# cjac/cmusphinx

Measured on AMD Instinct MI355X. Metric: decoded_frames_per_sec (full mode-4 decode, hub4-shaped CD-GMM 6144x8x39 + 20k-word lextrees + trigram; xRT = value/100/n_gpus), higher is better.
Workload: dtype f32-sub/f64-acc/int32-logadd (bit-exact), int32 Viterbi + word level; 1 GPU; lanes_per_gpu=512, engines_per_gpu=1

## Files before the change

### cmusphinx_amd/csrc/s3a_decoder_kernels.h

```cpp
#ifndef S3A_DECODER_KERNELS_H
#define S3A_DECODER_KERNELS_H
#include <hip/hip_runtime.h>
#include <stdlib.h>
#include <stdint.h>
#include <limits.h>
#include "s3a_device.h"
#include "s3a_structs.h"
#include "s3a_vit.h"
#include "s3a_scan.h"

#define WORST S3A_WORST
#define DBLOCK 256
#define S3A_ALD(p) __hip_atomic_load((p), __ATOMIC_RELAXED, __HIP_MEMORY_SCOPE_AGENT)
#define S3A_ALDU(p) __hip_atomic_load((p), __ATOMIC_RELAXED, __HIP_MEMORY_SCOPE_AGENT)
#define SCAN_LONG_LIST 16384
static inline int32_t scan_workgroups(int32_t rows, int chained)
{
    return (rows >= SCAN_LONG_LIST || chained) ? (rows + SCAN_THREADS - 1) / SCAN_THREADS : 1;
}
#define M3BLOCK 64
#define RSBLOCK 64
#define EVBLOCK_LONG_LIST 32768

struct FrameBeams {
// ... 1222 lines not shown
        c = lo;
        v = rootlist[calls[4 * c + 2] + (e - calls[4 * c + 3])];
    }
};

__device__ __forceinline__ void
d_dec_enter1(Entries ent, int32_t n_ent, const int32_t *__restrict__ calls,
             const int32_t *__restrict__ prob, const int32_t *__restrict__ sc, int32_t thresh,
             unsigned long long *key, int32_t *first,
        const int32_t BX, const int32_t BY)
{
    const int32_t e = BX * blockDim.x + threadIdx.x;
    int32_t idx, c;
    ent.locate_idx_wave(e < n_ent ? e : 0, idx, c);
    if (e >= n_ent) return;
    const int32_t scr = add32(calls[4 * c], ent.root_prob(idx, prob));
    if (scr < thresh) return;
    const int32_t v = ent.rootlist[idx];
    if (!(sc[NSV(v)] < scr)) return;
    atomicMax(&key[v], ((unsigned long long)((uint32_t)scr ^ 0x80000000u) << 32) | (uint32_t)(0x7fffffff - c));
    atomicMin(&first[v], c);
}

template <bool MAXOP>
__device__ __forceinline__ void
d_comsen_wave(int32_t n_cs, const int32_t *__restrict__ cs_need, int32_t stamp, const int32_t *__restrict__ cs_off,
              const int16_t *__restrict__ cs_list, uint8_t *sen_active, const int32_t *__restrict__ raw, int32_t *cs_val,
              int32_t cs0)
{
    const int32_t lane = threadIdx.x & 63, sub = lane >> 4, l16 = lane & 15;
    const int32_t mine = cs0 + lane;
    const unsigned long long mask = __ballot(mine < n_cs && cs_need[mine] == stamp);
    const int32_t n = __popcll(mask);
    for (int32_t k0 = 0; k0 < n; k0 += 4) {
        const int32_t k = k0 + sub;
        unsigned long long m = mask;
        for (int32_t i = 0; i < k && m; i++) m &= m - 1ull;
        const bool on = k < n;
        const int32_t cs = on ? cs0 + (__ffsll((long long)m) - 1) : 0;
        int32_t mx = INT_MIN;
        if (on)
            for (int32_t q = cs_off[cs] + l16, hi = cs_off[cs + 1]; q < hi; q += 16) {
                const int32_t id = cs_list[q];
                if (MAXOP) mx = max(mx, raw[id]); else sen_active[id] = 1;
            }
        if (MAXOP) {
#pragma unroll
            for (int o = 8; o > 0; o >>= 1) mx = max(mx, __shfl_xor(mx, o, 64));
            if (on && l16 == 0) cs_val[cs] = mx;
        }
    }
}

template <bool MAXOP, int U = 4>
__device__ __forceinline__ void
d_comsen_list(const int32_t *__restrict__ wl, int32_t n_w, const int32_t *__restrict__ cs_off, const int16_t *__restrict__ cs_list,
              uint8_t *sen_active, const int32_t *__restrict__ raw, int32_t *cs_val, int32_t grp, int32_t n_grp,
              const int32_t *__restrict__ cs_wt = NULL, uint32_t *actbits = NULL)
{
    const int32_t l16 = threadIdx.x & 15;
    for (int32_t j0 = 0; j0 < n_w; j0 += U * n_grp) {
        int32_t cs[U], lo[U], hi[U], mx[U];
        bool on[U];
#pragma unroll
        for (int u = 0; u < U; u++) { const int32_t j = j0 + u * n_grp + grp; on[u] = j < n_w; cs[u] = ((const __attribute__((address_space(1))) int32_t *)wl)[on[u] ? j : 0]; }
#pragma unroll
        for (int u = 0; u < U; u++) { const __attribute__((address_space(1))) int32_t *co = (const __attribute__((address_space(1))) int32_t *)cs_off; const int32_t a0 = co[cs[u]], a1 = co[cs[u] + 1]; lo[u] = on[u] ? a0 : 0; hi[u] = on[u] ? a1 : 0; mx[u] = INT_MIN; }
        for (int32_t q0 = 0; ; q0 += 32) {
            int32_t id[U][2];
            bool any = false;
#pragma unroll
            for (int u = 0; u < U; u++) {
#pragma unroll
                for (int h = 0; h < 2; h++) { const int32_t q = lo[u] + q0 + 16 * h + l16; const int32_t x = (int32_t)((const __attribute__((address_space(1))) int16_t *)cs_list)[q < hi[u] ? q : 0]; id[u][h] = q < hi[u] ? x : -1; }
                any = any || lo[u] + q0 < hi[u];
            }
            if (!any) break;
#pragma unroll
            for (int u = 0; u < U; u++)
#pragma unroll
                for (int h = 0; h < 2; h++)
                {
                    if (MAXOP) { const int32_t x = ((const __attribute__((address_space(1))) int32_t *)raw)[max(id[u][h], 0)]; if (id[u][h] >= 0) mx[u] = max(mx[u], x); }
                    else if (id[u][h] >= 0) { if (actbits) (void)__hip_atomic_fetch_or((__attribute__((address_space(3))) uint32_t *)&actbits[id[u][h] >> 5], 1u << (id[u][h] & 31), __ATOMIC_RELAXED, __HIP_MEMORY_SCOPE_WORKGROUP); else sen_active[id[u][h]] = 1; }
                }
        }
        if (MAXOP) {
#pragma unroll
            for (int u = 0; u < U; u++) {
#pragma unroll
                for (int o = 8; o > 0; o >>= 1) mx[u] = max(mx[u], __shfl_xor(mx[u], o, 64));
                if (on[u] && l16 == 0) ((__attribute__((address_space(1))) int32_t *)cs_val)[cs[u]] = cs_wt ? add32(mx[u], ((const __attribute__((address_space(1))) int32_t *)cs_wt)[cs[u]]) : mx[u];
            }
        }
    }
}

__device__ __forceinline__ void
mark_node_senones(int32_t v, const int32_t *__restrict__ ssid, const uint8_t *__restrict__ comp,
                  const int16_t *__restrict__ sseq, const int16_t *__restrict__ comsseq,
                  const int32_t *__restrict__ cs_off, const int16_t *__restrict__ cs_list, uint8_t *sen_active,
                  int32_t *cs_need = NULL, int32_t stamp = 0, int32_t ne = 3, int32_t *cs_wl = NULL, int32_t *cs_wn = NULL)
{
    const int32_t ss = ssid[v];
    if (comp[v] && cs_need && cs_wl) {
        for (int st = 0; st < ne; st++) {
            const int32_t cs = comsseq[ss * ne + st];
            if (atomicExch(&cs_need[cs], stamp) != stamp) cs_wl[atomicAdd(cs_wn, 1)] = cs;
        }
    }
    else if (comp[v] && cs_need) {
        if (ne == 3) {
#pragma unroll
            for (int st = 0; st < 3; st++) cs_need[comsseq[ss * 3 + st]] = stamp;
        }
        else for (int st = 0; st < ne; st++) cs_need[comsseq[ss * ne + st]] = stamp;
    }
    else if (comp[v] && ne != 3) {
        for (int st = 0; st < ne; st++) {
            const int32_t cs = comsseq[ss * ne + st];
            for (int32_t q = cs_off[cs]; q < cs_off[cs + 1]; q++) sen_active[cs_list[q]] = 1;
        }
    }
    else if (comp[v]) {
        int32_t lo[3], hi[3];
#pragma unroll
        for (int st = 0; st < 3; st++) {
            const int32_t cs = comsseq[ss * 3 + st];
            lo[st] = cs_off[cs]; hi[st] = cs_off[cs + 1];
        }
        while (lo[0] < hi[0] || lo[1] < hi[1] || lo[2] < hi[2]) {
            int32_t id[3][8];
#pragma unroll
            for (int st = 0; st < 3; st++)
#pragma unroll
                for (int u = 0; u < 8; u++) id[st][u] = (lo[st] + u < hi[st]) ? (int32_t)cs_list[lo[st] + u] : -1;
// ... 132 lines not shown
```

### cmusphinx_amd/csrc/s3a_utt.hip

```cpp
#include <hip/hip_runtime.h>
#include <stdint.h>
#include <stdlib.h>
#include <stdio.h>
#include <string.h>
#include <limits.h>
#include <vector>
#include <deque>
#include <atomic>
#include <mutex>
#include <algorithm>
#include <fcntl.h>
#include <unistd.h>
#include <sys/file.h>
#include <sys/stat.h>

#include "s3a_device.h"
#include "s3a_structs.h"
#include "s3a_decoder_kernels.h"
#include "s3a_gated.h"
#include "s3a_wordlevel.h"
#include "s3a_lm3g.h"
#include "s3a_dag.h"
#include "s3a_hostmem.h"
#include "s3a_kfplan.h"
#include "s3a_uttgeom.h"
#include "s3a_qsched.h"

#define S3A_AS1 __attribute__((address_space(1)))
#define S3A_AS3 __attribute__((address_space(3)))
typedef int s3a_v4i __attribute__((ext_vector_type(4)));
typedef int s3a_v2i __attribute__((ext_vector_type(2)));
template <class T> __device__ __forceinline__ S3A_AS1 T *GM(T *p) { return (S3A_AS1 T *)p; }
template <class T> __device__ __forceinline__ const S3A_AS1 T *GMC(const T *p) { return (const S3A_AS1 T *)p; }
template <class T> __device__ __forceinline__ const S3A_AS3 T *LM(const T *p) { return (const S3A_AS3 T *)p; }
__device__ __forceinline__ void lds_or(uint32_t *p, uint32_t v) { (void)__hip_atomic_fetch_or((S3A_AS3 uint32_t *)p, v, __ATOMIC_RELAXED, __HIP_MEMORY_SCOPE_WORKGROUP); }

struct ULane {
    int32_t *sc, *hist, *outs, *outh, *bests, *frame, *pos, *posf, *act[2], *nact[2], *turn, *selfemit, *cnt, *base,
        *best, *exits, *nexit, *first, *eflag, *hbin, *done, *ctot, *n0, *pstamp, *propf, *poswid, *posout, *scan_flag;
    unsigned long long *scan_agg, *scan_pre, *key;
    uint8_t *sen_act;
    int32_t *scr, *misc, *bstidx, *bstscr, *updatetime, *gpart;
    int32_t *cs_need, *cs_val;
    int32_t *cs_wl, *cs_wn;
    int32_t *posbest;
    uint32_t *senbits;
    int32_t *posps;
    int32_t *ent;
    uint8_t *pstamp8;
    int32_t *dynbeam;
    int32_t *claim;
    int32_t *plist, *pcnt;
    int32_t *win;
    uint8_t *winb;
    int32_t *ci_all;
    int32_t *heur_all;
    int32_t *hth_pos;
    int32_t *ph_scratch;
    UCtx *ctx;
    int32_t *pack;
    WLane w;
};

struct UShared {
    int32_t N, T, n_tmat, maxn, n_rootnodes, scan_chunks, pack_max_exits, gp_n, n_cs, n_pset_bytes;
    int32_t ne;
    const int32_t *node_base, *ssid, *tmatid, *wid, *prob, *child_off, *child, *par_off, *par, *tree_of, *rootlist, *tp,
        *rootnodes, *ps, *psof_off, *psof, *psmem_off, *psmem, *cs_off, *cs_wt, *rootprob;
    const uint8_t *comp;
    const int16_t *sseq, *comsseq, *cs_list;
    const int4 *node4;
    const int32_t *nodesen;
    const int4 *pshdr;
    const int4 *nodepk;
    const float4 *mean4, *prec4;
    const float *lrd;
    const int32_t *mixw;
    const uint16_t *tab16;
    uint32_t tab_size;
    int32_t lm_zero;
    double f, distfloor;
    int32_t D4, CP, Gpad, n_sen, n_ci_sen;
    const uint8_t *ncomp;
    const int16_t *cd2cisen;
    int32_t ds_ratio, ci_pbeam, ci_pbeam_tight, ptranskip;
    int32_t max_cd;
    float tighten;
    FrameBeams bm;
    int32_t pheurtype, pl_beam, pl_window, n_ci;
    const uint8_t *node_ci;
    const int16_t *sen2cimap;
    int32_t win_K;
    UCtx *ctx_all;
    int32_t *nact_all;
    const int32_t *fgbase;
};

#define LANE UCtx *ctx = S.ctx_all + blockIdx.z; const int32_t f = fg + *S.fgbase - ctx->f0;                         \
    if (f < 0 || f >= ctx->nfr || !ctx->active) return;                                                           \
    const int32_t cur = f & 1; const int32_t *nact_cur = S.nact_all + ((size_t)blockIdx.z * 2 + cur) * WL_MAXT;       \
    const ULane &L = lanes[blockIdx.z]; (void)cur; (void)nact_cur
#define SCR_ROW (S.win_K > 0 ? L.win + (size_t)(f % S.win_K) * S.n_sen : L.scr)

__device__ __forceinline__ FrameBeams
frame_beams(const UShared &S, int32_t cf)
{
    FrameBeams bm = S.bm;
    bm.phone_uses_wbeam = (S.ptranskip != 0 && (cf % S.ptranskip) == 0) ? 1 : 0;
    return bm;
}

struct UBegin { int32_t e0[10], lmc[5], n_pset; };

__device__ __forceinline__ void
// ... 564 lines not shown
            const int32_t sq = in ? senq[u] : S.n_ci_sen;
            actq[u] = actbits ? (uint8_t)((LM(actbits)[sq >> 5] >> (sq & 31)) & 1u) : L.sen_act[sq];
            if (!in) actq[u] = 0;
            ciq[u] = GMC(S.cd2cisen)[sq];
            senq[u] = sq;
        }
#pragma unroll
        for (int u = 0; u < 4; u++) {
            cisq[u] = GMC(row)[ciq[u]]; rowq[u] = GMC(row)[senq[u]]; nbq[u] = GMC(brow)[senq[u]];
            obq[u] = GMC(L.bstidx)[senq[u]]; utq[u] = GMC(L.updatetime)[senq[u]];
        }
#pragma unroll
        for (int u = 0; u < 4; u++) {
            if (!actq[u]) continue;
            const int32_t sen = senq[u];
            if (!actbits) L.sen_act[sen] = 0;
            const int32_t ci_scr = cisq[u];
            if (ci_scr >= thresh) {
                const int32_t bi = (int32_t)nbq[u];
                GM(L.bstidx)[sen] = bi == 255 ? S3A_NO_BSTIDX : bi;
                GM(L.updatetime)[sen] = f;
                rbest = max(rbest, rowq[u]); rns++; rng += (int32_t)GMC(S.ncomp)[sen];
                continue;
            }
            const int32_t bi = obq[u], ut = utq[u];
            if (bi == S3A_NO_BSTIDX || ut != f - 1) {
                GM(row)[sen] = ci_scr;
                rbest = max(rbest, ci_scr);
                continue;
            }
            const int32_t v = uw_one_gaussian<EXACT>(S, sen * S.CP + bi, ctx->feat + (size_t)f * S.D4 * 4);
            int32_t score = la(S3A_LOGPROB_ZERO, v);
            if (score <= S3A_LOGPROB_ZERO) score = S3A_LOGPROB_ZERO;
            row[sen] = score;
            rbest = max(rbest, score); rng++;
            if (is_skip) { L.bstidx[sen] = v > S3A_LOGPROB_ZERO ? bi : S3A_NO_BSTIDX; L.updatetime[sen] = f; }
        }
    }
#pragma unroll
    for (int o = 32; o > 0; o >>= 1) {
        rbest = max(rbest, __shfl_xor(rbest, o, 64)); rns += __shfl_xor(rns, o, 64); rng += __shfl_xor(rng, o, 64);
    }
    __syncthreads();
    if (ln == 0) { red[0][tid >> 6] = rbest; red[1][tid >> 6] = rns; red[2][tid >> 6] = rng; }
    __syncthreads();
    if (tid == 0 && bx < S.gp_n) {
        for (int w = 1; w < NT / 64; w++) { rbest = max(rbest, red[0][w]); rns += red[1][w]; rng += red[2][w]; }
        L.gpart[bx] = rbest;
        L.gpart[S.gp_n + bx] = rns;
        L.gpart[2 * S.gp_n + bx] = rng;
    }
}

template <bool EXACT>
__global__ void __launch_bounds__(256)
ku_select(const ULane *__restrict__ lanes, UShared S, int32_t fg, int32_t K)
{
    LANE;
    d_select<EXACT, 256>(L, S, ctx, f, L.win + (size_t)(f % K) * S.n_sen, L.winb + (size_t)(f % K) * S.n_sen, blockIdx.x, gridDim.x);
}

__global__ void __launch_bounds__(256)
ku_comsen_mark(const ULane *__restrict__ lanes, UShared S, int32_t fg)
{
    LANE;
    d_comsen_wave<false>(S.n_cs, L.cs_need, f, S.cs_off, S.cs_list, L.sen_act, (const int32_t *)NULL, (int32_t *)NULL,
                         (int32_t)blockIdx.x * 256 + (int32_t)(threadIdx.x & ~63));
}

#define UDB_MAXCI 1024
__global__ void __launch_bounds__(1024)
ku_dyn_ci_beam(const ULane *__restrict__ lanes, UShared S, int32_t fg)
{
    __shared__ int32_t s_occ[UDB_MAXCI], s_scr[UDB_MAXCI], s_ord[UDB_MAXCI], s_cut;
    LANE;
    const int32_t n_ci = S.n_ci_sen, tid = threadIdx.x;
    for (int32_t c = tid; c < n_ci; c += 1024) { s_occ[c] = 0; s_scr[c] = SCR_ROW[c]; }
    if (tid == 0) s_cut = INT_MAX;
    __syncthreads();
    for (int32_t s = n_ci + tid; s < S.n_sen; s += 1024)
        if (L.sen_act[s]) atomicAdd(&s_occ[S.cd2cisen[s]], 1);
    __syncthreads();
    for (int32_t c = tid; c < n_ci; c += 1024) {
        const int32_t v = s_scr[c];
        int32_t r = 0;
        for (int32_t c2 = 0; c2 < n_ci; c2++) { const int32_t v2 = s_scr[c2]; r += (v2 > v || (v2 == v && c2 < c)) ? 1 : 0; }
        s_ord[r] = c;
    }
    __syncthreads();
    const int32_t pbest = s_scr[s_ord[0]];
    for (int32_t r = tid; r < n_ci; r += 1024) {
        int32_t total = 0;
        for (int32_t r2 = 0; r2 <= r; r2++) total += s_occ[s_ord[r2]];
        if (total > S.max_cd) atomicMin(&s_cut, r);
    }
    __syncthreads();
    if (tid == 0) {
        int32_t beam = S.ci_pbeam;
        if (s_cut != INT_MAX) {
            const int32_t v = s_scr[s_ord[s_cut]];
            bool in_beam = true;
            for (int32_t r = 0; r <= s_cut && in_beam; r++) in_beam = s_scr[s_ord[r]] > add32(pbest, S.ci_pbeam);
            if (in_beam) beam = v - pbest;
        }
        if (f % S.ds_ratio != 0) beam = (int32_t)((float)beam * S.tighten);
        L.dynbeam[0] = beam;
// ... 568 lines not shown
#define KF_SENBITS 16384
#ifndef KF_ER
#define KF_ER 4
#endif
#ifndef KF_RL
#define KF_RL 8
#endif
#ifndef KF_SK
#define KF_SK 8
#endif
#ifndef KF_RK
#define KF_RK 4
#endif
#define KF_SETS 512
#define KF_TP_LDS 1024
#define KF_ENT 640
#define KF_BIG 256
static_assert(KF_NT == 512, "ku_frames: the word level's workgroup is the frame's workgroup");
enum { KF_WINDOW, KF_STATIC, KF_QUEUE };
#define KF_ST_WORDS 8
#define KF_OVERLAP_LEAD 128
#define KF_STAGES 2

union KfPool {
    struct { int32_t off[WL_MAXCALL], root[WL_MAXCALL], in[WL_MAXCALL], hist[WL_MAXCALL]; } e1;
    int32_t bin[NBIN];
    HistSortWs<KF_NT> hs;
    struct {
        union {
            int32_t rc[KF_WAVES][5 * 64];
            int32_t ent[KF_ENT][5];
        };
        int32_t mlo[KF_SETS], pre[KF_SETS + 1], big[KF_SETS], nbig, m_all;
        int32_t bmlo[KF_BIG], bnm[KF_BIG], bkp0[KF_BIG], bnp[KF_BIG];
        int32_t bnq[KF_BIG], bpre[KF_BIG + 1], bmpre[KF_BIG + 1], leg[KF_BIG], nleg;
        int32_t n_ent;
    } rs;
    struct { int32_t hdr[6 * WL_MAXT + 16], ex[3 * WL_LDS_EX]; } wl;
};

struct KfSh {
    KfPool pool;
    int32_t best[2 * WL_MAXT], acc[2 * WL_MAXT], pre[WL_MAXT + 1], red[KF_WAVES], dead, u, u2, dynbeam;
    int32_t fk, fk2;
    ULane Lc;
    int32_t nb[WL_MAXT + 1];
    int32_t seg[KF_MAXSEG + 1], ws[KF_WAVES + 1], gq[4];
    int32_t rk[KF_RK][KF_WAVES];
    uint32_t senbits[KF_SENBITS / 32];
    int32_t pstab[KF_PSTAB];
    int32_t ps_exact;
    uint32_t psbits[KF_PSBITS / 32];
    long long kacc[16];
    int32_t thr[4];
    int32_t tp[KF_TP_LDS];
    struct { const void *A; UCtx *ctx; int32_t *row; const uint8_t *brow; int32_t *bar_cnt; int32_t z, r, C, f, weak, bar_target, bar_local; } fa;
};

struct KfBar { int32_t *cnt; int32_t C, target; int32_t *dead; int32_t local; };

struct KfJob {
    int32_t mode, fg0, n_fr;
    int32_t n_utt;
    int32_t u0;
    const int32_t *order;
    int32_t stop_at;
    int32_t resume;
    int32_t *st_cur, *st_next;
    int32_t *lane_f, *lane_uq, *lane_stop;
    int32_t *next;
    int32_t *lane_u;
    const UCtx *stage;
    const long long *row0;
    int32_t *scores;
    const uint8_t *bests;
    int32_t *hdr, *words, *wcount;
    UHypPar P;
    UBegin B;
    int32_t n_word;
    int32_t ov;
    int32_t n1;
    const int32_t *q_ready;
    int32_t *lane_left;
    int32_t *n_resumed;
    const int32_t *f_ready;
    int32_t *n_inside;
};

__device__ __forceinline__ void
kf_barrier(KfBar &B)
{
    if (B.C == 1) { __syncthreads(); return; }
    if (B.local) asm volatile("s_waitcnt vmcnt(0) lgkmcnt(0)" ::: "memory");
    __syncthreads();
    B.target += B.C;
    if (threadIdx.x == 0 && !*B.dead) {
        if (!B.local) __builtin_amdgcn_fence(__ATOMIC_RELEASE, "agent");
        asm volatile("s_waitcnt vmcnt(0)" ::: "memory");
        (void)__hip_atomic_fetch_add(B.cnt, 1, __ATOMIC_RELAXED, __HIP_MEMORY_SCOPE_AGENT);
        int32_t spins = 0;
        while (__hip_atomic_load(B.cnt, __ATOMIC_RELAXED, __HIP_MEMORY_SCOPE_AGENT) < B.target) {
            __builtin_amdgcn_s_sleep(1);
            if (++spins > KF_SPIN_MAX) { *B.dead = 1; break; }
        }
        __builtin_amdgcn_fence(__ATOMIC_ACQUIRE, "agent");
    }
    __syncthreads();
}

__device__ __forceinline__ void
kf_locate(const int32_t *pre, int32_t T, int32_t g, int32_t &t, int32_t &i)
{
    t = 0;
    while (t + 1 < T && g >= pre[t + 1]) t++;
    i = g - pre[t];
}

template <int NE>
__device__ __forceinline__ int32_t
kf_hmm_eval(int32_t v, const int4 nd, const int32_t *__restrict__ nodesen, const int32_t *__restrict__ tp_g, const int32_t *tp_lds, const bool tp_in_lds,
            const int32_t *__restrict__ raw, const int32_t *raw_lds, const bool raw_in_lds, int32_t norm,
            const int32_t *__restrict__ cs_valw, int32_t *rec_all, int32_t cf, int32_t &w, int32_t &out)
{
    constexpr int NV = NE == 3 ? 2 : 3;
    S3A_AS1 s3a_v4i *rec = (S3A_AS1 s3a_v4i *)(rec_all + NSV(v));
    int32_t id[NE], tmat, wid_, comp;
    if (NE == 3) {
        id[0] = nd.x & 0xffff; id[1] = (int32_t)((uint32_t)nd.x >> 16); id[2] = nd.y & 0xffff;
        tmat = (int32_t)((uint32_t)nd.y >> 16); wid_ = nd.z; comp = nd.w & 1;
    }
    else {
        const s3a_v4i a5 = *(const S3A_AS1 s3a_v4i *)(nodesen + (size_t)v * 4);
        const int32_t h[5] = { a5.x & 0xffff, (int32_t)((uint32_t)a5.x >> 16), a5.y & 0xffff, (int32_t)((uint32_t)a5.y >> 16), a5.z & 0xffff };
#pragma unroll
        for (int st = 0; st < NE; st++) id[st] = h[st];
        tmat = nd.y; wid_ = nd.z; comp = nd.w;
    }
    int32_t e[NE], eg[NE];
    const S3A_AS1 int32_t *gsrc = GMC(comp ? cs_valw : raw);
// ... 133 lines not shown
    const int32_t n_ci = S.n_ci_sen, tid = threadIdx.x;
    for (int32_t c = tid; c < n_ci; c += NT) { s_occ[c] = 0; s_scr[c] = row[c]; }
    if (tid == 0) *s_cut = INT_MAX;
    __syncthreads();
    for (int32_t s = n_ci + tid; s < S.n_sen; s += NT)
        if ((senbits[s >> 5] >> (s & 31)) & 1u) atomicAdd(&s_occ[S.cd2cisen[s]], 1);
    __syncthreads();
    for (int32_t c = tid; c < n_ci; c += NT) {
        const int32_t v = s_scr[c];
        int32_t r = 0;
        for (int32_t c2 = 0; c2 < n_ci; c2++) { const int32_t v2 = s_scr[c2]; r += (v2 > v || (v2 == v && c2 < c)) ? 1 : 0; }
        s_ord[r] = c;
    }
    __syncthreads();
    const int32_t pbest = s_scr[s_ord[0]];
    for (int32_t r = tid; r < n_ci; r += NT) {
        int32_t total = 0;
        for (int32_t r2 = 0; r2 <= r; r2++) total += s_occ[s_ord[r2]];
        if (total > S.max_cd) atomicMin(s_cut, r);
    }
    __syncthreads();
    if (tid == 0) {
        int32_t beam = S.ci_pbeam;
        if (*s_cut != INT_MAX) {
            const int32_t v = s_scr[s_ord[*s_cut]];
            bool in_beam = true;
            for (int32_t r = 0; r <= *s_cut && in_beam; r++) in_beam = s_scr[s_ord[r]] > add32(pbest, S.ci_pbeam);
            if (in_beam) beam = v - pbest;
        }
        if (f % S.ds_ratio != 0) beam = (int32_t)((float)beam * S.tighten);
        *out = beam;
    }
    __syncthreads();
}

template <int NE, bool EXACT, bool HEUR = false>
__device__ __forceinline__ void
kf_frame(const ULane &L, const UShared &S, UCtx *ctx, const WLm &lm, const WDict &dict, const WPar &par, KfSh &sh, KfBar &B, int32_t z,
         int32_t r, int32_t C, int32_t f, int32_t *row, const uint8_t *brow, int32_t weak_flags)
{
    const int32_t weak_possible = weak_flags & 1, big_wl = weak_flags & 2;
    const int32_t tid = threadIdx.x, lane = tid & 63, wave = tid >> 6, T = S.T;
    const int32_t gtid = r * KF_NT + tid, gstride = C * KF_NT, gwave = r * KF_WAVES + wave, gwaves = C * KF_WAVES;
    long long t_prev = 0;
#define KF_STAMP(i) do { if (r == 0 && tid == 0) { const long long t_ = (long long)wall_clock64(); sh.kacc[i] += t_ - t_prev; t_prev = t_; } } while (0)
    const int32_t cur = f & 1;
    const int32_t *nact_cur = S.nact_all + ((size_t)z * 2 + cur) * WL_MAXT;
    const FrameBeams bm = frame_beams(S, f);
    const int32_t n_ent = ctx->n_ent, n_calls_all = ctx->n_calls, thresh = ctx->thresh;
    if (r == 0 && tid == 0) { t_prev = (long long)wall_clock64(); sh.kacc[13]++; }
    if (f == 0) {
        for (int32_t i = tid; i < KF_SENBITS / 32; i += KF_NT) sh.senbits[i] = 0u;
        if (C > 1 && r == 0) for (int32_t i = tid; i < KF_SENBITS / 32; i += KF_NT) L.senbits[i] = 0u;
        kf_barrier(B);
    }

    if (n_ent > 0) {
        const int32_t n_calls = min(n_calls_all, WL_MAXCALL), nf = f;
        if (tid < n_calls) {
            sh.pool.e1.in[tid] = ctx->calls[4 * tid]; sh.pool.e1.hist[tid] = ctx->calls[4 * tid + 1];
            sh.pool.e1.root[tid] = ctx->calls[4 * tid + 2]; sh.pool.e1.off[tid] = ctx->calls[4 * tid + 3];
        }
        if (r == 0 && tid < T) L.n0[tid] = L.nact[cur][tid];
        __syncthreads();
        const int32_t R = (((n_ent + gwaves - 1) / gwaves) + 63) & ~63, e_lo = gwave * R, e_hi = min(e_lo + R, n_ent);
        int32_t cntw = 0, c = 0;
        if (e_lo < e_hi) {
            int32_t lo = 0, hi = n_calls - 1;
            while (lo < hi) { const int32_t mid = (lo + hi + 1) >> 1; if (sh.pool.e1.off[mid] <= e_lo) lo = mid; else hi = mid - 1; }
            c = lo;
        }
        for (int32_t e0 = e_lo; e0 < e_hi; e0 += 64 * KF_ER) {
            int32_t scr[KF_ER], vv[KF_ER], cc[KF_ER], idx[KF_ER], s0[KF_ER];
            bool keep[KF_ER];
#pragma unroll
            for (int u = 0; u < KF_ER; u++) {
                const int32_t e = e0 + 64 * u + lane;
                keep[u] = false; scr[u] = INT_MIN; vv[u] = 0; cc[u] = c; idx[u] = 0;
                if (e < e_hi) {
                    while (c + 1 < n_calls && sh.pool.e1.off[c + 1] <= e) c++;
                    cc[u] = c; idx[u] = sh.pool.e1.root[c] + (e - sh.pool.e1.off[c]);
                }
            }
            int32_t rp[KF_ER];
#pragma unroll
            for (int u = 0; u < KF_ER; u++) { rp[u] = GMC(S.rootprob)[idx[u]]; vv[u] = GMC(S.rootlist)[idx[u]]; }
#pragma unroll
            for (int u = 0; u < KF_ER; u++) {
                if (e0 + 64 * u + lane < e_hi) scr[u] = add32(sh.pool.e1.in[cc[u]], rp[u]);
                keep[u] = e0 + 64 * u + lane < e_hi && scr[u] >= thresh;
            }
#pragma unroll
            for (int u = 0; u < KF_ER; u++) s0[u] = GMC(L.sc)[NSV(keep[u] ? vv[u] : __shfl(vv[u], 0, 64))];
#pragma unroll
            for (int u = 0; u < KF_ER; u++) {
                keep[u] = keep[u] && s0[u] < scr[u];
                const unsigned long long m = __ballot(keep[u]);
                if (keep[u]) {
                    const int32_t p_ = e_lo + cntw + __popcll(m & ((1ull << lane) - 1ull));
                    GM(L.eflag)[p_] = vv[u]; GM(L.ent)[2 * p_] = scr[u]; GM(L.ent)[2 * p_ + 1] = cc[u];
                    atomicMax(&L.key[vv[u]], ((unsigned long long)((uint32_t)scr[u] ^ 0x80000000u) << 32) | (uint32_t)(0x7fffffff - cc[u]));
                    atomicMin(&L.first[vv[u]], cc[u]);
                }
                cntw += __popcll(m);
            }
        }
// ... 96 lines not shown
            while (lo < hi) { const int32_t mid = (lo + hi + 1) >> 1; if (sh.seg[mid] <= 0) lo = mid; else hi = mid - 1; }
            p0 = lo * R;
        }
        const int32_t tg0 = ctx->groups[0], tg1 = ctx->n_groups > 1 ? ctx->groups[4] : ctx->groups[0];
        const int32_t n00 = L.n0[tg0], n01 = L.n0[tg1];
        for (int32_t i0 = gtid; i0 < P; i0 += 4 * gstride) {
            int32_t pq[4], vq[4], flq[4], fsq[4];
            unsigned long long kq[4];
            int4 aq[4];
#pragma unroll
            for (int u = 0; u < 4; u++) {
                const int32_t i = i0 + u * gstride;
                pq[u] = -1;
                if (i < P) {
                    int32_t lo = 0, hi = gwaves - 1;
                    while (lo < hi) { const int32_t mid = (lo + hi + 1) >> 1; if (sh.seg[mid] <= i) lo = mid; else hi = mid - 1; }
                    pq[u] = lo * R + (i - sh.seg[lo]);
                }
            }
#pragma unroll
            for (int u = 0; u < 4; u++) { const int32_t pk = pq[u] >= 0 ? pq[u] : p0; vq[u] = GMC(L.eflag)[pk]; flq[u] = GMC(L.ent)[2 * pk + 1]; }
#pragma unroll
            for (int u = 0; u < 4; u++) {
                kq[u] = S3A_ALD(&GM(L.key)[vq[u]]); fsq[u] = S3A_ALD(&GM(L.first)[vq[u]]);
                aq[u] = kf_mark_load<NE>(vq[u], NE == 3 ? (const int32_t *)S.nodepk : S.nodesen);
            }
#pragma unroll
            for (int u = 0; u < 4; u++) {
                if (pq[u] < 0) continue;
                const int32_t v = vq[u], fl = flq[u], c = fl & 127;
                const int32_t g = c >= c1 ? 1 : 0, t = g ? tg1 : tg0;
                if (fl & 128) {
                    const int32_t k = (g ? n01 : n00) + (fl >> 8) - (g ? gq0 : 0);
                    GM(L.act[cur])[sh.nb[t] + k] = v; { s3a_v2i o; o.x = k; o.y = nf; *(S3A_AS1 s3a_v2i *)(L.pos + PPX(v)) = o; }
                }
                const unsigned long long key = kq[u];
                const int32_t win_c = 0x7fffffff - (int32_t)(uint32_t)(key & 0xffffffffu);
                if (c == win_c) { GM(L.sc)[NSV(v)] = (int32_t)((uint32_t)(key >> 32) ^ 0x80000000u); GM(L.hist)[NSV(v)] = LM(sh.pool.e1.hist)[c]; }
                if (c == fsq[u]) GM(L.frame)[NSV(v)] = nf;
            }
            bool lq[4];
#pragma unroll
            for (int u = 0; u < 4; u++) lq[u] = pq[u] >= 0 && (flq[u] & 128) != 0;
            kf_mark_apply4<NE>(aq, lq, sh.senbits, L.cs_need, nf, L.cs_wl, L.cs_wn);
        }
    }
    kf_barrier(B);
    KF_STAMP(2);
    if (tid == 0) {
        int32_t a = 0;
        for (int32_t t = 0; t < T; t++) { sh.pre[t] = a; a += nact_cur[t]; }
        sh.pre[T] = a;
    }
    if (n_ent > 0) {
        const int32_t R = (((n_ent + gwaves - 1) / gwaves) + 63) & ~63, P = sh.seg[gwaves];
        for (int32_t i = gtid; i < P; i += gstride) {
            int32_t lo = 0, hi = gwaves - 1;
            while (lo < hi) { const int32_t mid = (lo + hi + 1) >> 1; if (sh.seg[mid] <= i) lo = mid; else hi = mid - 1; }
            const int32_t v = L.eflag[lo * R + (i - sh.seg[lo])];
            L.key[v] = 0ull; L.first[v] = INT_MAX;
        }
    }
    const int32_t n_csw = S3A_ALD(&L.cs_wn[0]);
#ifndef KF_CSU
#define KF_CSU 4
#endif
    d_comsen_list<false, KF_CSU>(L.cs_wl, n_csw, S.cs_off, S.cs_list, (uint8_t *)NULL, (const int32_t *)NULL, (int32_t *)NULL, gtid >> 4, gstride >> 4,
                         (const int32_t *)NULL, sh.senbits);
    if (C > 1) {
        __syncthreads();
        for (int32_t i = tid; i < KF_SENBITS / 32; i += KF_NT) if (sh.senbits[i]) atomicOr(&L.senbits[i], sh.senbits[i]);
    }
    kf_barrier(B);
    if (C > 1) {
        for (int32_t i = tid; i < KF_SENBITS / 32; i += KF_NT) sh.senbits[i] = S3A_ALDU(&L.senbits[i]);
        __syncthreads();
    }
    KF_STAMP(3);
    const int32_t n_tot = sh.pre[T];
    const bool hist_frame = n_tot > bm.maxhmmpf + (bm.maxhmmpf >> 1);
    {
        const int32_t g_all = max(1, min(USEL_G, min(S.gp_n, (S.n_sen - S.n_ci_sen + 255) / 256))), G = min(C, g_all);
        const bool dyn = S.max_cd < S.n_sen - S.n_ci_sen;
        if (dyn && r < G) kf_dyn_ci_beam<KF_NT>(S, f, row, sh.senbits, (int32_t *)&sh.pool, &sh.dynbeam);
        if (dyn && r == 0 && tid == 0) L.dynbeam[0] = sh.dynbeam;
        if (r < G) d_select<EXACT, KF_NT>(L, S, ctx, f, row, brow, r, G, sh.senbits, dyn ? &sh.dynbeam : (const int32_t *)NULL);
        if (r == 0 && tid >= G && tid < g_all) { L.gpart[tid] = INT_MIN; L.gpart[S.gp_n + tid] = 0; L.gpart[2 * S.gp_n + tid] = 0; }
    }
    kf_barrier(B);
    for (int32_t i = tid; i < KF_SENBITS / 32; i += KF_NT) sh.senbits[i] = 0u;
    if (C > 1 && r == 0) for (int32_t i = tid; i < KF_SENBITS / 32; i += KF_NT) L.senbits[i] = 0u;
    KF_STAMP(4);
    d_comsen_list<true, KF_CSU>(L.cs_wl, n_csw, S.cs_off, S.cs_list, (uint8_t *)NULL, row, L.cs_val, gtid >> 4, gstride >> 4, S.cs_wt);
    kf_barrier(B);
    KF_STAMP(5);
    {
        int32_t gb = INT_MIN;
        for (int32_t i = tid; i < S.gp_n; i += KF_NT) gb = max(gb, L.gpart[i]);
#pragma unroll
        for (int o = 32; o > 0; o >>= 1) gb = max(gb, __shfl_xor(gb, o, 64));
        if (lane == 0) sh.red[wave] = gb;
        if (tid < 2 * T) sh.acc[tid] = INT_MIN;
        if (r == 0 && tid == 0) L.cs_wn[0] = 0;
        const bool row_in_lds = (size_t)S.n_sen * 4 <= sizeof(KfPool);
        int32_t *row_lds = (int32_t *)&sh.pool;
        if (row_in_lds)
            for (int32_t i = tid; i < S.n_sen; i += KF_NT) row_lds[i] = row[i];
        __syncthreads();
        int32_t norm = max(L.misc[0], L.misc[5]);
        for (int w = 0; w < KF_WAVES; w++) norm = max(norm, sh.red[w]);
        const int32_t *act = L.act[cur];
        const bool tp_in_lds = S.n_tmat * NS_TPW(NE) <= KF_TP_LDS;
        int32_t t0 = -1, i0 = 0, b0 = 0, v0 = -1, t1 = -1, i1 = 0, b1 = 0, v1 = -1;
        int4 nd0 = make_int4(0, 0, 0, 0);
        {
            const int32_t ga = r * KF_NT + tid, gb_ = ga + gstride;
            if (ga < n_tot) { kf_locate(sh.pre, T, ga, t0, i0); b0 = sh.nb[t0]; v0 = act[b0 + i0]; }
            if (gb_ < n_tot) { kf_locate(sh.pre, T, gb_, t1, i1); b1 = sh.nb[t1]; v1 = act[b1 + i1]; }
            if (v0 >= 0) nd0 = (NE == 3 ? S.nodepk : S.node4)[v0];
        }
        for (int32_t g0 = r * KF_NT; g0 < n_tot; g0 += gstride) {
            int32_t t2 = -1, i2 = 0, b2 = 0, v2 = -1;
            const int32_t gc = g0 + 2 * gstride + tid;
            kf_locate(sh.pre, T, gc < n_tot ? gc : 0, t2, i2);
            b2 = sh.nb[t2];
            int4 nd1;
            { const s3a_v4i a = ((const S3A_AS1 s3a_v4i *)(NE == 3 ? S.nodepk : S.node4))[max(v1, 0)]; nd1 = make_int4(a.x, a.y, a.z, a.w); }
            {
                const int32_t vx = GMC(act)[b2 + i2];
                if (gc < n_tot) v2 = vx; else t2 = -1;
            }
            const int32_t t = t0;
            int32_t k = INT_MIN, w = -1;
            if (v0 >= 0) {
                int32_t out;
                k = kf_hmm_eval<NE>(v0, nd0, S.nodesen, S.tp, sh.tp, tp_in_lds, row, row_lds, row_in_lds, norm, L.cs_val, L.sc, f, w, out);
                GM(L.poswid)[b0 + i0] = w;
                GM(L.posout)[b0 + i0] = out;
                GM(L.posbest)[b0 + i0] = k;
                if (NE == 3) GM(L.posps)[b0 + i0] = (int32_t)((uint32_t)nd0.w >> 1);
            }
            unsigned long long todo = __ballot(t >= 0);
            while (todo) {
                const int32_t tt = __shfl(t, __ffsll((long long)todo) - 1, 64);
                const bool mine = t == tt;
                int32_t x = mine ? k : INT_MIN, y = (mine && w >= 0) ? k : INT_MIN;
#pragma unroll
                for (int o = 32; o > 0; o >>= 1) { x = max(x, __shfl_xor(x, o, 64)); y = max(y, __shfl_xor(y, o, 64)); }
                if (lane == 0) { atomicMax(&sh.acc[2 * tt], x); if (y != INT_MIN) atomicMax(&sh.acc[2 * tt + 1], y); }
                todo &= ~__ballot(mine);
            }
            t0 = t1; i0 = i1; b0 = b1; v0 = v1; nd0 = nd1;
            t1 = t2; i1 = i2; b1 = b2; v1 = v2;
        }
        __syncthreads();
        if (tid < 2 * T && sh.acc[tid] != INT_MIN) atomicMax(&L.best[tid], sh.acc[tid]);
    }
    kf_barrier(B);
    KF_STAMP(6);
// ... 502 lines not shown
kf_frame_call()
{
    KfSh &sh = g_kfsh<NE, EXACT>;
    const KfArgs *A = (const KfArgs *)kf_uniform_ptr(sh.fa.A);
    UCtx *ctx = kf_uniform_ptr(sh.fa.ctx);
    const int32_t z = __builtin_amdgcn_readfirstlane(sh.fa.z), r = __builtin_amdgcn_readfirstlane(sh.fa.r), C = __builtin_amdgcn_readfirstlane(sh.fa.C),
        f = __builtin_amdgcn_readfirstlane(sh.fa.f), weak = __builtin_amdgcn_readfirstlane(sh.fa.weak);
    KfBar B = { kf_uniform_ptr(sh.fa.bar_cnt), C, __builtin_amdgcn_readfirstlane(sh.fa.bar_target), &sh.dead, __builtin_amdgcn_readfirstlane(sh.fa.bar_local) };
    kf_frame<NE, EXACT>(sh.Lc, A->S, ctx, A->lm, A->dict, A->par, sh, B, z, r, C, f, kf_uniform_ptr(sh.fa.row), kf_uniform_ptr(sh.fa.brow), weak);
    if (threadIdx.x == 0) sh.fa.bar_target = B.target;
    __syncthreads();
}

#ifndef KF_OCC
#define KF_OCC 4
#endif

template <int NE, bool EXACT, bool HEUR = false>
__global__ void __launch_bounds__(KF_NT, KF_OCC)
ku_frames(const ULane *__restrict__ lanes, const KfArgs *__restrict__ A, int32_t n_lanes, int32_t C, int32_t *bar,
          int32_t weak_possible, int32_t local_ok)
{
    const UShared &S = A->S; const WLm &lm = A->lm; const WDict &dict = A->dict; const WPar &par = A->par; const KfJob &J = A->J;
    KfSh &sh = g_kfsh<NE, EXACT>;
    int32_t z, r;
    if (C == 1) { z = blockIdx.x; r = 0; }
    else { const int32_t b = blockIdx.x, xcd = b & 7, j = b >> 3; z = (j / C) * 8 + xcd; r = j % C; }
    if (z >= n_lanes) return;
    bool mid_left = false;
    if (J.ov == 2 && z < J.n1) {
        if (threadIdx.x == 0) {
            const int32_t was = atomicCAS(&J.lane_left[z], 0, 2);
            sh.u2 = was;
            if (was == 1 || was == 3) atomicAdd(J.n_resumed, 1);
            if (was == 3) atomicAdd(J.n_inside, 1);
        }
        __syncthreads();
        if (sh.u2 != 1 && sh.u2 != 3) return;
        mid_left = sh.u2 == 3;
        __builtin_amdgcn_fence(__ATOMIC_ACQUIRE, "agent");
        __syncthreads();
    }
    if (J.resume) {
        if (z >= __hip_atomic_load(&J.st_cur[2], __ATOMIC_RELAXED, __HIP_MEMORY_SCOPE_AGENT)) return;
        z = J.st_cur[KF_ST_WORDS + z];
    }
    const int32_t tid = threadIdx.x;
    static_assert(sizeof(ULane) % 4 == 0, "the lane's structure is copied to LDS word by word");
    for (int32_t i = tid; i < (int32_t)(sizeof(ULane) / 4); i += KF_NT) ((int32_t *)&sh.Lc)[i] = ((const int32_t *)&lanes[z])[i];
    const ULane &L = sh.Lc;
    UCtx *ctx = S.ctx_all + z;
    if (tid == 0) { sh.dead = 0; sh.fk = J.f_ready ? 0 : INT32_MAX; }
    if (tid < 16) sh.kacc[tid] = 0;
    for (int32_t i = tid; i < KF_SENBITS / 32; i += KF_NT) sh.senbits[i] = 0u;
    if (tid <= S.T) sh.nb[tid] = S.node_base[tid];
    if (S.n_tmat * NS_TPW(NE) <= KF_TP_LDS)
        for (int32_t i = tid; i < S.n_tmat * NS_TPW(NE); i += KF_NT) sh.tp[i] = S.tp[i];
    KfBar B = { bar + 2 * z, C, 0, &sh.dead, 0 };
    __syncthreads();
    if (C > 1) {
        if (tid == 0) atomicOr(bar + 2 * z + 1, 1 << (__builtin_amdgcn_s_getreg((31 << 11) | 20) & 15));
        kf_barrier(B);
        if (tid == 0) sh.u = __hip_atomic_load(bar + 2 * z + 1, __ATOMIC_RELAXED, __HIP_MEMORY_SCOPE_AGENT);
        __syncthreads();
        B.local = local_ok && __popc(sh.u) == 1;
        __syncthreads();
    }
    long long t_launch = (long long)wall_clock64();
    const int32_t mode = J.mode;
    const int32_t gtid = r * KF_NT + tid, gstride = C * KF_NT;
    bool resumed = J.resume != 0 || mid_left, handed = false, all_scored = false;
    if (resumed && C > 1) {
        if (r == 0) for (int32_t i = tid; i < KF_SENBITS / 32; i += KF_NT) L.senbits[i] = 0u;
        kf_barrier(B);
    }
    for (;;) {
        int32_t u = 0, f_lo = 0, f_hi = 0;
        size_t r0 = 0;
        if (resumed) {
            u = mode == KF_QUEUE ? J.lane_uq[z] : z;
            f_lo = J.lane_f[z]; f_hi = ctx->nfr;
            r0 = (size_t)J.row0[u];
            resumed = false;
        }
        else if (mode == KF_QUEUE) {
            if (r == 0 && tid == 0) {
                int32_t u_;
                if (J.q_ready) {
                    const int32_t ready = all_scored ? J.n_utt : __hip_atomic_load(J.q_ready, __ATOMIC_RELAXED, __HIP_MEMORY_SCOPE_AGENT);
                    u_ = __hip_atomic_load(J.next, __ATOMIC_RELAXED, __HIP_MEMORY_SCOPE_AGENT);
                    for (;;) {
                        if (u_ >= ready) { if (u_ < J.n_utt) u_ = -1; break; }
                        if (__hip_atomic_compare_exchange_strong(J.next, &u_, u_ + 1, __ATOMIC_RELAXED, __ATOMIC_RELAXED, __HIP_MEMORY_SCOPE_AGENT)) break;
                    }
                }
                else u_ = atomicAdd(J.next, 1);
                sh.u = u_;
                if (J.f_ready && (u_ >= J.n1 || all_scored)) sh.fk = INT32_MAX;
                if (C > 1) __hip_atomic_store(&J.lane_u[z], u_, __ATOMIC_RELAXED, __HIP_MEMORY_SCOPE_AGENT);
            }
            kf_barrier(B);
            if (r > 0 && tid == 0) sh.u = __hip_atomic_load(&J.lane_u[z], __ATOMIC_RELAXED, __HIP_MEMORY_SCOPE_AGENT);
            __syncthreads();
            u = sh.u;
            if (u < 0) {
                if (tid == 0) { sh.kacc[12] += (long long)wall_clock64() - t_launch; sh.kacc[14]++; }
                __syncthreads();
                if (tid < 16) { ctx->kacc[tid] += sh.kacc[tid]; sh.kacc[tid] = 0; }
                if (tid == 0 && J.ov == 1) {
                    ctx->kdbg[0] = t_launch; ctx->kdbg[1] = (long long)wall_clock64();
                    ctx->kdbg[2] = (long long)__builtin_amdgcn_s_getreg((31 << 11) | 4); ctx->kdbg[3] = (long long)__builtin_amdgcn_s_getreg((31 << 11) | 20);
                }
                asm volatile("s_waitcnt vmcnt(0)" ::: "memory");
                __syncthreads();
                if (tid == 0) {
                    __builtin_amdgcn_fence(__ATOMIC_RELEASE, "agent");
                    sh.u2 = atomicCAS(&J.lane_left[z], 0, 1);
                }
                __syncthreads();
                if (sh.u2 == 0) return;
                all_scored = true;
                t_launch = (long long)wall_clock64();
                continue;
            }
            if (u >= J.n_utt || sh.dead) break;
            if (J.q_ready) __builtin_amdgcn_fence(__ATOMIC_ACQUIRE, "agent");
            u = J.order[J.u0 + u];
            if (r == 0 && tid == 0 && J.lane_uq) J.lane_uq[z] = u;
            d_lane_begin(L, S, J.B, z, J.stage + u, gtid, gstride, r == 0, tid, KF_NT);
            kf_barrier(B);
            f_hi = ctx->nfr;
            r0 = (size_t)J.row0[u];
        }
        else if (mode == KF_STATIC) { f_hi = ctx->nfr; r0 = (size_t)J.row0[z]; }
        else { const int32_t f0 = ctx->f0; f_lo = max(0, J.fg0 - f0); f_hi = min(ctx->nfr, J.fg0 + J.n_fr - f0); }
        for (int32_t f = f_lo; f < f_hi; f++) {
            if (!((volatile UCtx *)ctx)->active || sh.dead) break;
            const bool ask = f >= sh.fk;
            if (J.stop_at > 0 || ask) {
                if (r == 0 && tid == 0) {
                    const int32_t st = J.stop_at > 0 ? __hip_atomic_load(&J.st_cur[1], __ATOMIC_RELAXED, __HIP_MEMORY_SCOPE_AGENT) : 0;
                    sh.u2 = st;
                    if (C > 1) __hip_atomic_store(&J.lane_stop[z], st, __ATOMIC_RELAXED, __HIP_MEMORY_SCOPE_AGENT);
                    if (ask) sh.fk2 = __hip_atomic_load(J.f_ready, __ATOMIC_RELAXED, __HIP_MEMORY_SCOPE_AGENT);
                }
                kf_barrier(B);
                if (C > 1 && r > 0 && tid == 0) sh.u2 = __hip_atomic_load(&J.lane_stop[z], __ATOMIC_RELAXED, __HIP_MEMORY_SCOPE_AGENT);
                if (C > 1) __syncthreads();
                const int32_t stop = sh.u2;
                if (ask) {
                    const int32_t F = sh.fk2;
                    __builtin_amdgcn_fence(__ATOMIC_ACQUIRE, "agent");
                    if (tid == 0) sh.fk = F;
                    if (f >= F) {
                        if (tid == 0) { sh.kacc[12] += (long long)wall_clock64() - t_launch; sh.kacc[14]++; J.lane_f[z] = f; }
                        __syncthreads();
                        if (tid < 16) { ctx->kacc[tid] += sh.kacc[tid]; sh.kacc[tid] = 0; }
                        if (tid == 0 && J.ov == 1) {
                            ctx->kdbg[0] = t_launch; ctx->kdbg[1] = (long long)wall_clock64();
                            ctx->kdbg[2] = (long long)__builtin_amdgcn_s_getreg((31 << 11) | 4); ctx->kdbg[3] = (long long)__builtin_amdgcn_s_getreg((31 << 11) | 20);
                        }
                        asm volatile("s_waitcnt vmcnt(0)" ::: "memory");
                        __syncthreads();
                        if (tid == 0) {
                            __builtin_amdgcn_fence(__ATOMIC_RELEASE, "agent");
                            sh.u2 = atomicCAS(&J.lane_left[z], 0, 3);
                        }
                        __syncthreads();
                        if (sh.u2 == 0) return;
                        __builtin_amdgcn_fence(__ATOMIC_ACQUIRE, "agent");
                        if (tid == 0) sh.fk = INT32_MAX;
                        all_scored = true;
                        t_launch = (long long)wall_clock64();
                    }
                }
                if (stop) {
                    if (r == 0 && tid == 0) {
                        J.lane_f[z] = f;
                        J.st_next[KF_ST_WORDS + atomicAdd(&J.st_next[2], 1)] = z;
                        atomicAdd(&J.st_next[0], 1);
                    }
                    handed = true;
                    break;
                }
            }
            int32_t *row = mode == KF_WINDOW ? L.win + (size_t)(f % S.win_K) * S.n_sen : J.scores + (r0 + f) * S.n_sen;
            const uint8_t *brow = mode == KF_WINDOW ? L.winb + (size_t)(f % S.win_K) * S.n_sen : J.bests + (r0 + f) * S.n_sen;
#if KF_CALL
            if (tid == 0) {
                sh.fa.A = A; sh.fa.ctx = ctx; sh.fa.row = row; sh.fa.brow = brow; sh.fa.bar_cnt = B.cnt; sh.fa.z = z; sh.fa.r = r; sh.fa.C = C; sh.fa.f = f;
                sh.fa.weak = weak_possible; sh.fa.bar_target = B.target; sh.fa.bar_local = B.local;
            }
            __syncthreads();
            kf_frame_call<NE, EXACT>();
            B.target = sh.fa.bar_target;
#else
            kf_frame<NE, EXACT, HEUR>(L, S, ctx, lm, dict, par, sh, B, z, r, C, f, row, brow, weak_possible);
#endif
        }
        if (handed) break;
        if (mode != KF_QUEUE) break;
        if (r == 0 && tid < 16 && tid != 12 && tid != 14) { ctx->kacc[tid] += sh.kacc[tid]; sh.kacc[tid] = 0; }
        static_assert(3 * WL_LDS_EX >= UH_IDS, "d_hyp's backtrace ids borrow the word level's exit area");
        if (r == 0) d_hyp<KF_NT>(L, ctx, lm, dict, J.P, J.hdr + (size_t)u * UH_N, J.words, J.wcount, sh.pool.wl.ex);
        kf_barrier(B);
        d_lane_end(L, S, z, ctx->err != 0, J.n_word, gtid, gstride);
        kf_barrier(B);
    }
    if (J.stop_at > 0 && !handed && r == 0 && tid == 0) {
        const int32_t left = atomicSub(&J.st_cur[0], 1) - 1;
        if (left <= J.stop_at && left > 0) __hip_atomic_store(&J.st_cur[1], 1, __ATOMIC_RELAXED, __HIP_MEMORY_SCOPE_AGENT);
    }
    if (r == 0 && tid == 0) { sh.kacc[12] += (long long)wall_clock64() - t_launch; sh.kacc[14]++; }
    if (r == 0 && tid < 16) ctx->kacc[tid] += sh.kacc[tid];
    if (r == 0 && tid == 0 && ((J.mode == KF_WINDOW && J.fg0 == 512) || J.ov == 1 || (J.ov == 2 && z >= J.n1))) {
        ctx->kdbg[0] = t_launch; ctx->kdbg[1] = (long long)wall_clock64();
        ctx->kdbg[2] = (long long)__builtin_amdgcn_s_getreg((31 << 11) | 4); ctx->kdbg[3] = (long long)__builtin_amdgcn_s_getreg((31 << 11) | 20);
    }
    if (sh.dead && tid == 0) { ctx->err |= WL_E_SCAN; ctx->active = 0; }
}

#define LANE_W const ULane &L = lanes[blockIdx.z]; UCtx *ctx = L.ctx; const int32_t f = fg - ctx->f0;               \
    if (f < 0 || f >= ctx->nfr || !ctx->active) return
__global__ void __launch_bounds__(WL_THREADS)
ku_wl_p2(const ULane *__restrict__ lanes, WLm lm, WDict dict, WPar par, int32_t fg)
{
    LANE_W;
    d_wl_big_p2(L.w, ctx, L.pack, lm, dict, par, f, blockIdx.x, gridDim.x);
}
__global__ void __launch_bounds__(WL_THREADS)
ku_wl_p3(const ULane *__restrict__ lanes, WDict dict, WPar par, int32_t fg)
{
    LANE_W;
    d_wl_big_p3(L.w, ctx, L.pack, dict, par, f, blockIdx.x, gridDim.x);
}
__global__ void __launch_bounds__(WL_THREADS)
ku_wl_p4a(const ULane *__restrict__ lanes, WPar par, int32_t fg)
{
    LANE_W;
    d_wl_big_p4a(L.w, ctx, L.pack, par, f, blockIdx.x, gridDim.x);
}
__global__ void __launch_bounds__(WL_THREADS)
ku_wl_p4b(const ULane *__restrict__ lanes, WPar par, int32_t fg)
{
    LANE_W;
    d_wl_big_p4b(L.w, ctx, L.pack, par, f, blockIdx.x, gridDim.x);
}
__global__ void __launch_bounds__(WL_THREADS)
ku_wl_p5(const ULane *__restrict__ lanes, WDict dict, WPar par, int32_t fg)
{
    LANE_W;
    d_wl_big_p5(L.w, ctx, L.pack, dict, par, f, blockIdx.x, gridDim.x);
}
__global__ void __launch_bounds__(WL_THREADS)
ku_wl_finish(const ULane *__restrict__ lanes, WLm lm, WDict dict, WPar par, int32_t fg)
{
    LANE_W;
    d_wl_big_finish(L.w, ctx, L.pack, lm, dict, par, f);
}

__global__ void __launch_bounds__(WL_THREADS)
ku_wordlevel_only(const ULane *__restrict__ lanes, WLm lm, WDict dict, WPar par)
{
    __shared__ int32_t s_hdr[6 * WL_MAXT + 16], s_ex[3 * WL_LDS_EX];
    const ULane &L = lanes[blockIdx.z];
    if (!L.ctx->active) return;
    const int32_t hdr = 6 * par.T + 16;
// ... 241 lines not shown
    std::vector<int32_t> h_lwid, h_fillpen, h_last_ci, h_tree_type;
    std::vector<uint8_t> h_is_filler;
    std::vector<HostLane> lane;
    ULane *d_lanes;
    int32_t *d_lcmap;
    std::vector<int32_t> h_lcmap;
    int device;
    UgShape shape;
    UgEngine geom;
    struct FrameGeom { int32_t n, hist_sort_launch; UgFrame fr; UgScore win; };
    std::deque<FrameGeom> frame_geoms;
    UgCall call;
    const void *kf_asked;
    hipStream_t stream;
    int32_t n_utt;
    double last_decode_ms;
    int32_t prof_every;
    struct ProfEv { int32_t cls; hipEvent_t a, b; };
    std::vector<ProfEv> prof_ev;
    double prof_us[24];
    int64_t prof_n[24];
    hipEvent_t ev0, ev1;
    int32_t *d_dbg;
    int32_t times;
    UCtx *h_ctx_dn;
    int32_t *d_hyp_hdr, *h_hyp_hdr;
    int32_t *d_hyp_words, *h_hyp_words;
    int32_t hyp_wcap;
    UCtx *h_ctx_up;
    int32_t n_pset;
    s3a_dagpass_t *dag;
    int32_t keep_tables;
    int32_t tables_fetched, fstat_fetched;
    int32_t *d_fgbase;
    struct FrameGraph { int32_t n, frames; hipGraphExec_t exec; UShared S; };
    std::vector<FrameGraph> graphs;
    int32_t q_n;
    std::vector<int32_t> q_nfr;
    s3a_grow<float> q_feat;
    s3a_grow<UCtx> q_ctx;
    s3a_grow<int32_t> q_sched;
    s3a_grow<int32_t> q_hdr;
    s3a_grow<int32_t> q_words, q_words_pin;
    s3a_grow<int32_t> q_dio;
    s3a_grow<int32_t> q_dw, q_dw_pin;
    int32_t q_dag;
    int32_t q_keep_lat;
    struct QLat { s3a_lat_info_t info; std::vector<s3a_lat_node_t> nodes; std::vector<s3a_lat_link_t> links; int32_t have; };
    std::vector<QLat> q_lat;
    int32_t *d_kfbar;
    int32_t kf_last_c;
    int32_t kf_counted;
    int32_t *d_kfnext;
    void *d_kfargs, *h_kfargs;
    int32_t kf_arg_at;
    s3a_grow<int32_t> sb_scores; s3a_grow<uint8_t> sb_bests;
    size_t sb_rows_max;
    s3a_grow<int32_t> kf_order;
    int32_t kf_shared;
    int32_t *d_kfrelay;
    int32_t kf_n_relay;
    s3a_grow<UwGroup> sb_gdesc;
    s3a_grow<long long> sb_row0;
    std::vector<hipEvent_t> kf_evs;
    int32_t kf_ev_n, kf_n_score, kf_n_frames;
    double kf_score_ms, kf_frames_ms;
    hipStream_t kf_stream2;
    hipEvent_t kf_ov_ev[3];
    int32_t *d_kfleft;
    int32_t kf_overlapped;
    int32_t kf_lead;
};

enum { KFN_COUNTER = 0, KFN_Q_READY = 1, KFN_RESUMED = 2, KFN_F_READY = 3, KFN_INSIDE = 4, KFN_LANE = 16 };

static std::atomic<int> g_kf_live[64];

static std::mutex g_kf_lock_mu;
static int g_kf_lock_fd[64], g_kf_lock_n[64], g_kf_lock_own[64];
static bool
kf_device_lock(int dev)
{
    std::lock_guard<std::mutex> lk(g_kf_lock_mu);
    if (g_kf_lock_n[dev]++ > 0) return g_kf_lock_own[dev] != 0;
    char bus[64] = "", path[160];
    if (hipDeviceGetPCIBusId(bus, sizeof bus, dev) != hipSuccess) snprintf(bus, sizeof bus, "dev%d", dev);
    for (char *c = bus; *c; c++) if (*c == ':' || *c == '/' || *c == '.') *c = '_';
    snprintf(path, sizeof path, "/dev/shm/cmusphinx_amd.kf.%s.lock", bus);
    const int fd = open(path, O_CREAT | O_RDWR | O_CLOEXEC, 0666);
    g_kf_lock_fd[dev] = fd;
    if (fd < 0) { g_kf_lock_own[dev] = 1; return true; }
    (void)fchmod(fd, 0666);
    g_kf_lock_own[dev] = flock(fd, LOCK_EX | LOCK_NB) == 0 ? 1 : 0;
    return g_kf_lock_own[dev] != 0;
}
static void
kf_device_unlock(int dev)
{
    std::lock_guard<std::mutex> lk(g_kf_lock_mu);
    if (--g_kf_lock_n[dev] > 0) return;
    if (g_kf_lock_fd[dev] >= 0) { (void)flock(g_kf_lock_fd[dev], LOCK_UN); (void)close(g_kf_lock_fd[dev]); }
    g_kf_lock_fd[dev] = -1; g_kf_lock_own[dev] = 0; g_kf_lock_n[dev] = 0;
}

static int32_t
fill32(hipStream_t st, int32_t *p, int32_t v, size_t n)
// ... 225 lines not shown
            for (int32_t k = 0; k < proto->n_lc[t]; k++) {
                const int32_t p = proto->lc[t][k];
                if (p < 0 || p >= cfg->n_ci) continue;
                ud->h_lcmap[((size_t)t * (cfg->n_ci + 1) + p) * 2] = proto->rootbuf_base[t] + proto->lcroot_off[t][k];
                ud->h_lcmap[((size_t)t * (cfg->n_ci + 1) + p) * 2 + 1] = proto->lcroot_off[t][k + 1] - proto->lcroot_off[t][k];
            }
        }
        else {
            for (int32_t p = 0; p <= cfg->n_ci; p++) {
                ud->h_lcmap[((size_t)t * (cfg->n_ci + 1) + p) * 2] = proto->rootbuf_base[t] + proto->lcroot_off[t][0];
                ud->h_lcmap[((size_t)t * (cfg->n_ci + 1) + p) * 2 + 1] = proto->lcroot_off[t][1] - proto->lcroot_off[t][0];
            }
        }
    }
    {
        int32_t *p0 = NULL, *p1 = NULL, *p2 = NULL;
        uint8_t *p3 = NULL;
        DM(ud->mem, p0, (size_t)cfg->n_word * 4); DM(ud->mem, p1, (size_t)cfg->n_word * 4); DM(ud->mem, p2, (size_t)cfg->n_word * 4); DM(ud->mem, p3, (size_t)cfg->n_word);
        ud->dict.lwid = p0; ud->dict.fillpen = p1; ud->dict.last_ci = p2; ud->dict.is_filler = p3;
        ud->dict.n_word = cfg->n_word; ud->dict.n_ci = cfg->n_ci;
        if (hipMemcpy(p0, cfg->lwid, (size_t)cfg->n_word * 4, hipMemcpyHostToDevice) != hipSuccess
            || hipMemcpy(p1, cfg->fillpen, (size_t)cfg->n_word * 4, hipMemcpyHostToDevice) != hipSuccess
            || hipMemcpy(p2, cfg->last_ci, (size_t)cfg->n_word * 4, hipMemcpyHostToDevice) != hipSuccess
            || hipMemcpy(p3, cfg->is_filler, (size_t)cfg->n_word, hipMemcpyHostToDevice) != hipSuccess) {
            s3a_set_error("s3a_uttdec_init: upload failed");
            goto fail;
        }
        UPV(ud->mem, ud->d_lcmap, ud->h_lcmap);
    }
    {
        WPar &P = ud->par;
        memset(&P, 0, sizeof P);
        P.wbeam = cfg->wbeam_vh; P.bghist = cfg->bghist; P.maxwpf = cfg->maxwpf; P.maxhist = cfg->maxhistpf;
        P.wordend = cfg->wordend_beam; P.n_lextree = cfg->n_lextree; P.epl = cfg->epl; P.T = T; P.hmmbeam = cfg->hmmbeam;
        for (int32_t t = 0; t < T; t++) P.tree_type[t] = cfg->tree_type[t];
        P.lcmap = ud->d_lcmap;
    }

    S.win_K = ud->geom.win_K;
    ud->times = O.times;
    ud->lane.resize(n_lanes);
    for (auto &hl : ud->lane) memset((void *)&hl, 0, sizeof hl);
    if (T > WL_MAXT) { s3a_set_error("s3a_uttdec_init: more than %d lextrees", WL_MAXT); goto fail; }
    DM(ud->mem, ud->S.ctx_all, sizeof(UCtx) * n_lanes);
    DM(ud->mem, ud->S.nact_all, (size_t)n_lanes * 2 * WL_MAXT * 4);
    DM(ud->mem, ud->d_fgbase, 64);
    if (hipMemset(ud->d_fgbase, 0, 64) != hipSuccess) goto fail;
    ud->S.fgbase = ud->d_fgbase;
    ud->sb_rows_max = O.score_rows_max > 0 ? (size_t)O.score_rows_max : 0;
    if (ud->geom.persist) {
        DM(ud->mem, ud->d_kfnext, (size_t)(KFN_LANE + n_lanes) * 4);
        DM(ud->mem, ud->d_kfargs, sizeof(KfArgs) * KF_ARG_SLOTS);
        if (!ud->mem.pin(ud->h_kfargs, sizeof(KfArgs) * KF_ARG_SLOTS)) { s3a_set_error("s3a_uttdec_init: pinned allocation failed"); goto fail; }
        DM(ud->mem, ud->d_kfbar, (size_t)n_lanes * 8);
        if (hipMemset(ud->d_kfbar, 0, (size_t)n_lanes * 8) != hipSuccess) goto fail;
        DM(ud->mem, ud->d_kfrelay, ((size_t)(KF_STAGES + 1) * (KF_ST_WORDS + n_lanes) + (size_t)3 * n_lanes) * 4);
        DM(ud->mem, ud->d_kfleft, (size_t)3 * n_lanes * 4);
        if (ud->device >= 0 && ud->device < 64) { g_kf_live[ud->device]++; ud->kf_counted = 1; ud->kf_shared = kf_device_lock(ud->device) ? 0 : 1; }
    }
    ud->hyp_wcap = max_frames + 4;
    if (!ud->mem.pin(ud->h_ctx_up, sizeof(UCtx) * n_lanes) || !ud->mem.pin(ud->h_ctx_dn, sizeof(UCtx) * n_lanes)
        || !ud->mem.pin(ud->h_hyp_hdr, ((size_t)n_lanes * UH_N + 1) * 4) || !ud->mem.pin(ud->h_hyp_words, (size_t)n_lanes * ud->hyp_wcap * 6 * 4)) { s3a_set_error("s3a_uttdec_init: pinned allocation failed"); goto fail; }
    memset(ud->h_ctx_dn, 0, sizeof(UCtx) * n_lanes);
    DM(ud->mem, ud->d_hyp_hdr, ((size_t)n_lanes * UH_N + 1) * 4);
    DM(ud->mem, ud->d_hyp_words, (size_t)n_lanes * ud->hyp_wcap * 6 * 4);
    if (hipMemset(ud->S.nact_all, 0, (size_t)n_lanes * 2 * WL_MAXT * 4) != hipSuccess
        || hipMemset(ud->S.ctx_all, 0, sizeof(UCtx) * n_lanes) != hipSuccess) goto fail;
    for (int32_t z = 0; z < n_lanes; z++) {
        HostLane &hl = ud->lane[z];
        hl.ls = s3a_lexsearch_clone(proto, (void *)ud->stream);
        hl.sc = s3a_scorer_init_private(g, cd2cisen, n_sen, n_ci_sen, ds_ratio, cond_ds, ci_pbeam, tighten_factor, max_cd);
        if (!hl.ls || !hl.sc) goto fail;
        if (z == 0) {
            S.gp_n = ud->shape.gp_n = hl.sc->gp_n;
            S.ci_pbeam = hl.sc->ci_pbeam;
            S.ci_pbeam_tight = (int32_t)((float)hl.sc->ci_pbeam * hl.sc->tighten_factor);
            S.max_cd = max_cd; S.tighten = hl.sc->tighten_factor;
            S.ncomp = hl.sc->ncomp_d;
            S.cd2cisen = hl.sc->cd2cisen_d;
        }
        s3a_lexsearch_t *ls = hl.ls;
        ULane &u = hl.d;
        u.sc = ls->d_sc; u.hist = ls->d_hist; u.outs = ls->d_outs; u.outh = ls->d_outh; u.bests = ls->d_bests;
        u.frame = ls->d_frame; u.pos = ls->d_pos; u.posf = ls->d_posf; u.act[0] = ls->d_act[0]; u.act[1] = ls->d_act[1];
        ls->mem.release(ls->d_nact[0]); ls->mem.release(ls->d_nact[1]);
        ls->d_nact[0] = ud->S.nact_all + ((size_t)z * 2) * WL_MAXT; ls->d_nact[1] = ud->S.nact_all + ((size_t)z * 2 + 1) * WL_MAXT;
        u.nact[0] = ls->d_nact[0]; u.nact[1] = ls->d_nact[1]; u.turn = ls->d_turn; u.selfemit = ls->d_selfemit;
        u.cnt = ls->d_cnt; u.base = ls->d_cand; u.best = ls->d_best; u.exits = ls->d_exit; u.nexit = ls->d_nexit;
        u.first = ls->d_first; u.eflag = ls->d_eflag; u.hbin = ls->d_hbin; u.done = ls->d_done; u.ctot = ls->d_ctot;
        u.n0 = ls->d_n0; u.pstamp = ls->d_pstamp; u.propf = ls->d_candf; u.poswid = ls->d_poswid; u.posout = ls->d_posout;
        u.scan_flag = ls->d_scan_flag; u.scan_agg = ls->d_scan_agg; u.scan_pre = ls->d_scan_pre; u.key = ls->d_key;
        u.sen_act = hl.sc->act_d; u.scr = hl.sc->scr_d; u.misc = hl.sc->misc_d; u.bstidx = hl.sc->bstidx_d;
        u.bstscr = hl.sc->bstscr_d; u.updatetime = hl.sc->updatetime_d; u.gpart = hl.sc->gpart_d;
        DM(ud->mem, u.cs_need, (size_t)(cs->n_comstate + 1) * 4); DM(ud->mem, u.cs_val, (size_t)(cs->n_comstate + 1) * 4); DM(ud->mem, u.dynbeam, 16);
        DM(ud->mem, u.cs_wl, (size_t)(cs->n_comstate + 1) * 4); DM(ud->mem, u.cs_wn, 16); u.ent = ls->d_ent; DM(ud->mem, u.posbest, (size_t)(proto->N + 64) * 4); DM(ud->mem, u.posps, (size_t)(proto->N + 64) * 4);
        DM(ud->mem, u.senbits, KF_SENBITS / 8); if (hipMemset(u.senbits, 0, KF_SENBITS / 8) != hipSuccess) goto fail;
        if (hipMemset(u.cs_wn, 0, 16) != hipSuccess) goto fail; DM(ud->mem, u.pstamp8, (size_t)proto->n_pset + 64); S.n_pset_bytes = proto->n_pset + 64;
        DM(ud->mem, u.plist, (size_t)(proto->N + 64) * 4); DM(ud->mem, u.pcnt, 16); DM(ud->mem, u.claim, (size_t)(proto->N + 64) * 4);
        if (hipMemset(u.pcnt, 0, 16) != hipSuccess) goto fail;
        if (hipMemset(u.pstamp8, 0xff, (size_t)proto->n_pset + 64) != hipSuccess) goto fail;
        if (S.win_K > 0) {
            DM(ud->mem, u.win, (size_t)S.win_K * n_sen * 4); DM(ud->mem, u.winb, (size_t)S.win_K * n_sen);
            if (fill32(ud->stream, u.gpart, INT_MIN, (size_t)max(S.gp_n, 0)) != S3A_OK
                || fill32(ud->stream, u.gpart + max(S.gp_n, 0), 0, (size_t)2 * max(S.gp_n, 0)) != S3A_OK) goto fail;
        }
        if (fill32(ud->stream, u.cs_need, -1, (size_t)cs->n_comstate + 1) != S3A_OK) goto fail;
        u.ctx = ud->S.ctx_all + z;
        DM(ud->mem, u.pack, (size_t)(6 * T + 16 + 3 * proto->pack_max_exits) * 4);
        if (wlane_alloc(ud->mem, u.w, ud->vh_cap, max_frames, ud->ex_cap, ud->cand_cap, ud->new_cap, cfg->n_word, ud->stream) != S3A_OK) goto fail;
        hl.h_ctx = ud->h_ctx_dn + z;
        if (!ud->mem.pin(hl.h_st, 16 * 4) || !ud->mem.pin(hl.h_fstat, (size_t)max_frames * 8 * 4)) {
            s3a_set_error("s3a_uttdec_init: pinned allocation failed");
            goto fail;
        }
    }
    {
        std::vector<ULane> tmp(n_lanes);
        for (int32_t z = 0; z < n_lanes; z++) tmp[z] = ud->lane[z].d;
        DM(ud->mem, ud->d_lanes, sizeof(ULane) * n_lanes);
        if (hipMemcpy(ud->d_lanes, tmp.data(), sizeof(ULane) * n_lanes, hipMemcpyHostToDevice) != hipSuccess) goto fail;
    }
    if (hipStreamSynchronize(ud->stream) != hipSuccess) goto fail;
    return ud;
fail:
    s3a_uttdec_free(ud);
    return NULL;
}

static int32_t
lane_scrub(s3a_uttdec_t *ud, int32_t z)
{
    HostLane &hl = ud->lane[z];
    int32_t rc;
    if (!hl.dirty) return S3A_OK;
    const WLane &w = hl.d.w;
    const size_t hs = (size_t)w.hmask + 1;
    if ((rc = s3a_lexsearch_reset(hl.ls)) != S3A_OK) return rc;
    HIPCHK(hipMemsetAsync(w.hkey, 0, hs * 8, ud->stream)); HIPCHK(hipMemsetAsync(w.hbest, 0, hs * 8, ud->stream));
    HIPCHK(hipMemsetAsync(w.hfirst, 0xff, hs * 4, ud->stream));
    if ((rc = fill32(ud->stream, w.wfirst, INT_MAX, ud->cfg.n_word)) != S3A_OK || (rc = fill32(ud->stream, w.wbest, INT_MIN, ud->cfg.n_word)) != S3A_OK) return rc;
    hl.dirty = 0;
    return S3A_OK;
}

static int32_t
utt_context(const s3a_uttdec_t *ud, UCtx &x, const float *d_feat, int32_t nfr, int32_t scan_epoch, int32_t f0, int32_t utt)
{
    const s3a_wordlevel_cfg_t &c = ud->cfg;
    memset(&x, 0, sizeof x);
// ... 252 lines not shown
    if (hold) HIPCHK(hipEventRecord(ud->kf_ov_ev[2], s1));
    HIPCHK(hipStreamWaitEvent(s2, ud->kf_ov_ev[0], 0));
    size_t n_sc = P.script.size();
    while (n_sc > 0 && P.script[n_sc - 1].op != KFP_SCORE) n_sc--;
    for (size_t i = 0; i < P.script.size(); i++) {
        const KfStep &st = P.script[i];
        if (st.op == KFP_SCORE) {
            if ((rc = uw_launch(ud, 0, 0, false, ud->sb_gdesc.d + st.a, (int32_t)(st.b - st.a), true, s2)) != S3A_OK) return rc;
            ud->kf_n_score++;
        }
        else if (!hold) HIPCHK(hipMemsetD32Async((hipDeviceptr_t)(st.op == KFP_F_READY ? f_ready : q_ready), (int32_t)st.a, 1, s2));
        if (i + 1 == n_sc) kf_mark(ud, s2);
    }
    if (hold) {
        HIPCHK(hipStreamWaitEvent(s2, ud->kf_ov_ev[2], 0));
        if (P.f_ready0 > 0 && P.f_ready0 < INT32_MAX) HIPCHK(hipMemsetD32Async((hipDeviceptr_t)f_ready, INT32_MAX, 1, s2));
        HIPCHK(hipMemsetD32Async((hipDeviceptr_t)q_ready, J.n_utt, 1, s2));
    }
    J.ov = 2;
    if ((rc = kf_launch_c(ud, n, J, 1, s2)) != S3A_OK) return rc;
    HIPCHK(hipEventRecord(ud->kf_ov_ev[1], s2));
    HIPCHK(hipStreamWaitEvent(s1, ud->kf_ov_ev[1], 0));
    return S3A_OK;
}

static int32_t
kf_launch_chain(s3a_uttdec_t *ud, int32_t n, KfJob J, const KfPlan *ov = NULL)
{
    ud->call.alone = kf_alone(ud);
    const UgKf G = ug_kf(ud->shape, ud->geom, ud->call, n, ov != NULL);
    const int32_t C0 = G.c0, n_st = G.n_st, st_c[KF_STAGES] = { G.st_c1, G.st_c2 }, st_cap[KF_STAGES] = { G.st_cap1, G.st_cap2 }, W = KF_ST_WORDS + ud->n_lanes;
    if (n_st == 0) return ov ? kf_launch_overlapped(ud, n, J, *ov) : kf_launch_c(ud, n, J, C0);
    HIPCHK(hipMemsetAsync(ud->d_kfrelay, 0, ((size_t)(KF_STAGES + 1) * W + (size_t)3 * ud->n_lanes) * 4, ud->stream));
    HIPCHK(hipMemsetD32Async((hipDeviceptr_t)ud->d_kfrelay, n, 1, ud->stream));
    J.lane_f = ud->d_kfrelay + (size_t)(KF_STAGES + 1) * W; J.lane_uq = J.lane_f + ud->n_lanes; J.lane_stop = J.lane_uq + ud->n_lanes;
    int32_t rc = S3A_OK;
    for (int32_t k = 0; k <= n_st && rc == S3A_OK; k++) {
        J.resume = k > 0; J.stop_at = k < n_st ? st_cap[k] : 0;
        J.st_cur = ud->d_kfrelay + (size_t)k * W; J.st_next = ud->d_kfrelay + (size_t)(k + 1) * W;
        if (k == 0 && ov) rc = kf_launch_overlapped(ud, n, J, *ov);
        else rc = kf_launch_c(ud, k == 0 ? n : st_cap[k - 1], J, k == 0 ? C0 : st_c[k - 1]);
    }
    ud->kf_n_relay = n_st;
    return rc;
}

static int32_t
enqueue_block(s3a_uttdec_t *ud, int32_t n, int32_t fg0, int32_t nf)
{
    int32_t rc = uw_launch(ud, n, fg0, false);
    if (rc != S3A_OK) return rc;
    KfJob J;
    memset(&J, 0, sizeof J);
    J.mode = KF_WINDOW; J.fg0 = fg0; J.n_fr = nf;
    ud->kf_n_score++; ud->kf_n_frames++;
    return kf_launch_c(ud, n, J, ug_kf_choose_c(ud->shape, ud->geom, kf_alone(ud), n));
}

static void
kf_mark(s3a_uttdec_t *ud, hipStream_t st = NULL)
{
    if ((size_t)ud->kf_ev_n >= ud->kf_evs.size()) {
        hipEvent_t e = NULL;
        if (hipEventCreate(&e) != hipSuccess) return;
        ud->kf_evs.push_back(e);
    }
    (void)hipEventRecord(ud->kf_evs[ud->kf_ev_n++], st ? st : ud->stream);
}

static void
kf_collect(s3a_uttdec_t *ud)
{
    ud->kf_score_ms = ud->kf_frames_ms = 0.0;
    if (ud->kf_overlapped && ud->kf_ev_n == 4) {
        float a = 0.0f, b = 0.0f;
        if (hipEventElapsedTime(&a, ud->kf_evs[0], ud->kf_evs[2]) == hipSuccess) ud->kf_score_ms = a;
        if (hipEventElapsedTime(&b, ud->kf_evs[1], ud->kf_evs[3]) == hipSuccess) ud->kf_frames_ms = b;
        ud->kf_ev_n = 0;
        return;
    }
    for (int32_t i = 0; i + 2 < ud->kf_ev_n; i += 3) {
        float a = 0.0f, b = 0.0f;
        if (hipEventElapsedTime(&a, ud->kf_evs[i], ud->kf_evs[i + 1]) == hipSuccess) ud->kf_score_ms += a;
        if (hipEventElapsedTime(&b, ud->kf_evs[i + 1], ud->kf_evs[i + 2]) == hipSuccess) ud->kf_frames_ms += b;
    }
    ud->kf_ev_n = 0;
}

static size_t
sb_budget_rows(const s3a_uttdec_t *ud)
{
    size_t fr = 0, tot = 0;
    if (hipMemGetInfo(&fr, &tot) != hipSuccess) return 0;
    const size_t per_row = (size_t)ud->S.n_sen * 5, rows = (fr / 2 + ud->sb_scores.cap * per_row) / per_row;
    return ud->sb_rows_max > 0 ? min(rows, ud->sb_rows_max) : rows;
}

static int32_t
sb_reserve(s3a_uttdec_t *ud, size_t rows, size_t groups, size_t n_utt)
{
    const size_t S_ = (size_t)ud->S.n_sen;
    if (rows > ud->sb_scores.cap) {
        const size_t grow = rows + rows / 16 + 64;
        ud->sb_scores.clear(ud->mem); ud->sb_bests.clear(ud->mem);
        if (ud->sb_scores.reserve(ud->mem, S3A_GROW_DEV, rows, grow, S_ * 4) != S3A_OK || ud->sb_bests.reserve(ud->mem, S3A_GROW_DEV, rows, grow, S_) != S3A_OK) {
            ud->sb_scores.clear(ud->mem);
            s3a_set_error("s3a_uttdec: the score buffer (%zu rows of %zu senones) does not fit the device", grow, S_);
            return S3A_ENOMEM;
        }
    }
    int32_t rc;
    if ((rc = q_reserve(ud, ud->sb_gdesc, S3A_GROW_DEV | S3A_GROW_PIN, groups, "score groups")) != S3A_OK) return rc;
    if ((rc = q_reserve(ud, ud->sb_row0, S3A_GROW_DEV | S3A_GROW_PIN, n_utt + 1, "score rows")) != S3A_OK) return rc;
    return S3A_OK;
}

static int32_t
sb_load(s3a_uttdec_t *ud, const KfPlan &P, const float *const *feat_dev)
{
    const size_t S_ = (size_t)ud->S.n_sen, n_utt = P.order.size();
    const int32_t DP = ud->S.D4 * 4;
    int32_t rc;
    if ((rc = sb_reserve(ud, P.max_rows, P.groups.size(), n_utt)) != S3A_OK) return rc;
    for (size_t g = 0; g < P.groups.size(); g++) {
        const KfGroup &k = P.groups[g];
        UwGroup &gr = ud->sb_gdesc.h[g];
        gr.feat = feat_dev[k.utt] + (size_t)k.first * DP;
        gr.win = ud->sb_scores.d + (size_t)k.row * S_;
        gr.winb = ud->sb_bests.d + (size_t)k.row * S_;
        gr.nv = k.frames; gr.pad = 0;
    }
    for (size_t u = 0; u < n_utt; u++) ud->sb_row0.h[u] = (long long)P.row0[u];
    HIPCHK(hipMemcpyAsync(ud->sb_gdesc.d, ud->sb_gdesc.h, P.groups.size() * sizeof(UwGroup), hipMemcpyHostToDevice, ud->stream));
    HIPCHK(hipMemcpyAsync(ud->sb_row0.d, ud->sb_row0.h, n_utt * 8, hipMemcpyHostToDevice, ud->stream));
    return S3A_OK;
}

static int32_t
sb_score(s3a_uttdec_t *ud, size_t g0, size_t n_g, bool companion = false, hipStream_t st = NULL)
{
    companion = companion || s3a_variants()->uw_companion != 0;
    for (size_t g = 0; g < n_g; g += SB_PIECE) {
        const int32_t rc = uw_launch(ud, 0, 0, false, ud->sb_gdesc.d + g0 + g, (int32_t)min((size_t)SB_PIECE, n_g - g), companion, st);
        if (rc != S3A_OK) return rc;
        ud->kf_n_score++;
    }
    return S3A_OK;
}

static int32_t
kf_static_group(s3a_uttdec_t *ud, int32_t m, const long long *row0, size_t g0, size_t n_g)
{
    int32_t rc;
    kf_mark(ud);
    if ((rc = sb_score(ud, g0, n_g)) != S3A_OK) return rc;
    kf_mark(ud);
    KfJob J;
    memset(&J, 0, sizeof J);
    J.mode = KF_STATIC; J.row0 = row0; J.scores = ud->sb_scores.d; J.bests = ud->sb_bests.d;
    if ((rc = kf_launch_chain(ud, m, J)) != S3A_OK) return rc;
    ud->kf_n_frames++;
    kf_mark(ud);
    return S3A_OK;
}

static int32_t
kf_decode_static(s3a_uttdec_t *ud, int32_t n_utt, const KfPlan &P)
{
    std::vector<const float *> fd((size_t)n_utt);
    for (int32_t z = 0; z < n_utt; z++) fd[z] = ud->h_ctx_up[z].feat;
    int32_t rc;
    if ((rc = sb_load(ud, P, fd.data())) != S3A_OK) return rc;
    ud->kf_n_score = ud->kf_n_frames = 0;
    return kf_static_group(ud, n_utt, ud->sb_row0.d, 0, P.groups.size());
}

static int32_t
kf_decode_queue(s3a_uttdec_t *ud, int32_t n_utt, const float *const *feat_dev, const int32_t *n_frames, const UBegin &B, const UHypPar &P,
                int32_t *wcount)
{
    const size_t budget = sb_budget_rows(ud);
    const s3a_variants_t *va = s3a_variants();
    int32_t n1 = ug_kf(ud->shape, ud->geom, ud->call, ud->n_lanes, 0).n1;
    const auto plan = [&](int32_t first) {
        int32_t lead_g, round_g;
        ug_kf_rounds(ud->call, first, &lead_g, &round_g);
        return kf_plan(n_utt, n_frames, KFP_BUDGET, budget, va->kf_queue_in_order != 0, first, lead_g, round_g, va->kf_overlap_whole != 0);
    };
    KfPlan K = plan(n1);
    if (K.max_rows > budget) { s3a_set_error("s3a_uttdec_decode_queue: an utterance's scores (%zu rows) do not fit the device", K.max_rows); return S3A_ENOMEM; }
    if (K.n1 > 0) {
        bool have = ud->kf_stream2 || hipStreamCreateWithFlags(&ud->kf_stream2, hipStreamNonBlocking) == hipSuccess;
        if (!have) { (void)hipGetLastError(); ud->kf_stream2 = NULL; }
        for (auto &e : ud->kf_ov_ev)
            if (have && !e && hipEventCreateWithFlags(&e, hipEventDisableTiming) != hipSuccess) { (void)hipGetLastError(); e = NULL; have = false; }
        if (!have) K = plan(0);
    }
    n1 = K.n1;
    int32_t rc;
    if ((rc = q_reserve(ud, ud->kf_order, S3A_GROW_DEV | S3A_GROW_PIN, (size_t)n_utt, "queue order")) != S3A_OK) return rc;
    ud->kf_overlapped = n1 > 0 ? 1 : 0;
    ud->kf_lead = K.lead;
    if (n1 > 0 && ud->kf_arg_at % KF_ARG_SLOTS + 2 + KF_STAGES > KF_ARG_SLOTS) {
        HIPCHK(hipStreamSynchronize(ud->stream));
        HIPCHK(hipStreamSynchronize(ud->kf_stream2));
        ud->kf_arg_at = 0;
    }
    if ((rc = sb_load(ud, K, feat_dev)) != S3A_OK) return rc;
    memcpy(ud->kf_order.h, K.order.data(), (size_t)n_utt * 4);
    HIPCHK(hipMemcpyAsync(ud->kf_order.d, ud->kf_order.h, (size_t)n_utt * 4, hipMemcpyHostToDevice, ud->stream));
    ud->kf_n_score = ud->kf_n_frames = 0;
    for (size_t k = 0; k + 1 < K.cut.size(); k++) {
        const int32_t u0 = K.cut[k], nu = K.cut[k + 1] - K.cut[k];
        kf_mark(ud);
        if (n1 > 0) rc = sb_score(ud, 0, K.g_lead, K.lead > 0);
        else rc = sb_score(ud, K.g_at[k], K.g_at[k + 1] - K.g_at[k]);
        if (rc != S3A_OK) return rc;
        kf_mark(ud);
        if (n1 > 0) {
            HIPCHK(hipMemsetAsync(ud->d_kfnext, 0, KFN_LANE * 4, ud->stream));
            HIPCHK(hipMemsetD32Async((hipDeviceptr_t)(ud->d_kfnext + KFN_Q_READY), n1, 1, ud->stream));
            if (K.lead > 0) HIPCHK(hipMemsetD32Async((hipDeviceptr_t)(ud->d_kfnext + KFN_F_READY), K.f_ready0, 1, ud->stream));
            HIPCHK(hipMemsetAsync(ud->d_kfleft, 0, (size_t)ud->n_lanes * 4, ud->stream));
        }
        else HIPCHK(hipMemsetAsync(ud->d_kfnext + KFN_COUNTER, 0, 4, ud->stream));
        KfJob J;
        memset(&J, 0, sizeof J);
        J.mode = KF_QUEUE; J.n_utt = nu; J.u0 = u0; J.order = ud->kf_order.d; J.next = ud->d_kfnext + KFN_COUNTER; J.lane_u = ud->d_kfnext + KFN_LANE; J.stage = ud->q_ctx.d;
        J.row0 = ud->sb_row0.d; J.scores = ud->sb_scores.d; J.bests = ud->sb_bests.d;
        J.hdr = ud->q_hdr.d; J.words = ud->q_words.d; J.wcount = wcount; J.P = P; J.B = B; J.n_word = ud->cfg.n_word;
        if ((rc = kf_launch_chain(ud, min(ud->n_lanes, nu), J, n1 > 0 ? &K : NULL)) != S3A_OK) return rc;
        ud->kf_n_frames++;
        kf_mark(ud);
    }
    return S3A_OK;
}

static int32_t
graph_block_frames(const s3a_uttdec_t *ud)
{
    return ud->S.win_K > 0 ? ud->S.win_K : 8;
}

static int32_t
graph_for(s3a_uttdec_t *ud, int32_t n, hipGraphExec_t *out)
{
    const int32_t G = graph_block_frames(ud);
    for (auto &g : ud->graphs)
        if (g.n == n && g.frames == G && memcmp(&g.S, &ud->S, sizeof(UShared)) == 0) { *out = g.exec; return S3A_OK; }
    if (ud->S.win_K > 0) {
        const int32_t rc0 = uw_launch(ud, n, 0, true);
        if (rc0 != S3A_OK) return rc0;
    }
    hipGraph_t graph = NULL;
    hipGraphExec_t exec = NULL;
    if (hipStreamBeginCapture(ud->stream, hipStreamCaptureModeThreadLocal) != hipSuccess) { s3a_set_error("s3a_uttdec: hipStreamBeginCapture failed: %s", hipGetErrorString(hipGetLastError())); return S3A_EHIP; }
    int32_t rc = S3A_OK;
    for (int32_t j = 0; j < G && rc == S3A_OK; j++) rc = enqueue_frame(ud, frame_geom(ud, n).fr, j, false);
    if (rc == S3A_OK) hipLaunchKernelGGL(ku_advance, dim3(1), dim3(64), 0, ud->stream, ud->d_fgbase, G);
    if (hipStreamEndCapture(ud->stream, &graph) != hipSuccess || !graph) { s3a_set_error("s3a_uttdec: hipStreamEndCapture failed: %s", hipGetErrorString(hipGetLastError())); return S3A_EHIP; }
    if (rc != S3A_OK) { (void)hipGraphDestroy(graph); return rc; }
    if (hipGraphInstantiate(&exec, graph, NULL, NULL, 0) != hipSuccess || !exec) { (void)hipGraphDestroy(graph); s3a_set_error("s3a_uttdec: hipGraphInstantiate failed: %s", hipGetErrorString(hipGetLastError())); return S3A_EHIP; }
    (void)hipGraphDestroy(graph);
    s3a_uttdec_s::FrameGraph fgr;
    fgr.n = n; fgr.frames = G; fgr.exec = exec; fgr.S = ud->S;
    ud->graphs.push_back(fgr);
    *out = exec;
    return S3A_OK;
}

static int32_t
lane_fetch_fstat(s3a_uttdec_t *ud, int32_t z)
{
    HostLane &hl = ud->lane[z];
    HIPCHK(hipMemcpyAsync(hl.h_fstat, hl.d.w.fstat, (size_t)hl.nfr * 8 * 4, hipMemcpyDeviceToHost, ud->stream));
    return S3A_OK;
}

static int32_t
lane_fetch_table(s3a_uttdec_t *ud, int32_t z)
{
// ... 127 lines not shown
        }
        else if (window) rc = enqueue_block(ud, n, f, min(step, f_end - f));
        else rc = enqueue_frame(ud, *G, f, ud->prof_every > 0 && f % ud->prof_every == 0);
    }
    if (rc == S3A_OK) rc = event(f_end);
    if (graph && rc == S3A_OK && hipMemsetAsync(ud->d_fgbase, 0, 4, ud->stream) != hipSuccess) rc = S3A_EHIP;
    return rc;
}

static int32_t
lane_begin(s3a_uttdec_t *ud, int32_t z, const float *feat, int32_t nfr, int32_t feat_stride, bool feat_on_device)
{
    HostLane &hl = ud->lane[z];
    const int32_t D4x4 = ud->S.D4 * 4;
    int32_t rc;
    if (nfr <= 0 || nfr > ud->max_frames) { s3a_set_error("s3a_uttdec_decode: %d frames (1..%d)", nfr, ud->max_frames); return S3A_EINVAL; }
    const float *d_feat_use = feat;
    if (!feat_on_device) {
        const size_t need = (size_t)nfr * D4x4;
        const size_t grow = (size_t)min(ud->max_frames, max(nfr + nfr / 2, 1024)) * D4x4;
        if (hl.feat_d.reserve(ud->mem, S3A_GROW_DEV, need, grow) != S3A_OK) { s3a_set_error("s3a_uttdec_decode: feature buffer"); return S3A_ENOMEM; }
        if (hl.feat_h.reserve(ud->mem, S3A_GROW_PIN, need, grow) != S3A_OK) { s3a_set_error("s3a_uttdec_decode: pinned feature buffer"); return S3A_ENOMEM; }
        stage_features(ud, hl.feat_h.h, feat, nfr, feat_stride);
        HIPCHK(hipMemcpyAsync(hl.feat_d.d, hl.feat_h.h, need * 4, hipMemcpyHostToDevice, ud->stream));
        d_feat_use = hl.feat_d.d;
    }
    else if (feat_stride != D4x4) {
        s3a_set_error("s3a_uttdec_decode_dev: device features must have rows of %d floats (zero padded)", D4x4);
        return S3A_EINVAL;
    }
    hl.nfr = nfr;
    if ((rc = lane_scrub(ud, z)) != S3A_OK) return rc;
    lane_host_reset(hl);
    UCtx &x = *hl.h_ctx;
    if ((rc = utt_context(ud, x, d_feat_use, nfr, hl.epoch, 0, -1)) != S3A_OK) return rc;
    hl.epoch += nfr + 1;
    ud->h_ctx_up[z] = x;
    return S3A_OK;
}

static int32_t
uttdec_decode(s3a_uttdec_t *ud, int32_t n_utt, const float *const *feat, const int32_t *n_frames,
              int32_t feat_stride, bool feat_on_device)
{
    if (!ud || n_utt <= 0 || n_utt > ud->n_lanes || !feat || !n_frames || feat_stride < ud->veclen) {
        s3a_set_error("s3a_uttdec_decode: bad arguments (%d utterances, %d lanes)", n_utt, ud ? ud->n_lanes : 0);
        return S3A_EINVAL;
    }
    HIPCHK(hipSetDevice(ud->device));
    call_facts(ud, false, n_utt);
    int32_t rc, maxT = 0;
    ud->q_n = 0;
    ud->kf_n_score = ud->kf_n_frames = ud->kf_last_c = ud->kf_n_relay = ud->kf_overlapped = 0;
    double tm[6] = { 0, 0, 0, 0, 0, 0 };
    auto now = []() { struct timespec ts; clock_gettime(CLOCK_MONOTONIC, &ts); return ts.tv_sec + 1e-9 * ts.tv_nsec; };
    tm[0] = now();
    for (int32_t z = 0; z < n_utt; z++) {
        if ((rc = lane_begin(ud, z, feat[z], n_frames[z], feat_stride, feat_on_device)) != S3A_OK) return rc;
        maxT = max(maxT, n_frames[z]);
    }
    hipLaunchKernelGGL(ku_lanes_end, dim3(8, 2 * ud->S.T, n_utt), dim3(256), 0, ud->stream, ud->d_lanes, ud->S, (const int32_t *)NULL, 0);
    hipLaunchKernelGGL(ku_lanes_begin, dim3(32, 1, n_utt), dim3(256), 0, ud->stream, ud->d_lanes, ud->S, utt_begin_par(ud), (const int32_t *)NULL, (const int32_t *)NULL, (const UCtx *)NULL);
    HIPCHK(hipGetLastError());
    HIPCHK(hipMemcpyAsync(ud->S.ctx_all, ud->h_ctx_up, sizeof(UCtx) * n_utt, hipMemcpyHostToDevice, ud->stream));
    if ((rc = enqueue_pheur_tables(ud, maxT, n_utt, NULL)) != S3A_OK) return rc;
    if ((rc = call_events(ud, "s3a_uttdec_decode")) != S3A_OK) return rc;
    tm[1] = now();
    if (hipEventRecord(ud->ev0, ud->stream) != hipSuccess) rc = S3A_EHIP;
    KfPlan P;
    int32_t route = ug_route(ud->shape, ud->geom, ud->call, 0, 0);
    if (route == UG_ROUTE_KF_STATIC) {
        P = kf_plan(n_utt, n_frames, KFP_ONE, 0, true, 0, 0, 0, false);
        route = ug_route(ud->shape, ud->geom, ud->call, (int64_t)P.max_rows, (int64_t)sb_budget_rows(ud));
    }
    if (rc == S3A_OK && route == UG_ROUTE_KF_STATIC) rc = kf_decode_static(ud, n_utt, P);
    else if (rc == S3A_OK) rc = enqueue_steps(ud, "s3a_uttdec_decode", route, n_utt, maxT, [](int32_t) { return (int32_t)S3A_OK; });
    if (rc == S3A_OK && hipEventRecord(ud->ev1, ud->stream) != hipSuccess) rc = S3A_EHIP;
    tm[2] = now();
    if (rc == S3A_OK) {
        const UHypPar P = utt_hyp_par(ud, (int32_t)min((long long)ud->n_lanes * ud->hyp_wcap, (long long)INT_MAX));
        if (hipMemsetAsync(ud->d_hyp_hdr + (size_t)n_utt * UH_N, 0, 4, ud->stream) != hipSuccess) rc = S3A_EHIP;
        hipLaunchKernelGGL(ku_hyp, dim3(n_utt), dim3(UH_T), 0, ud->stream, ud->d_lanes, ud->lm->d, ud->dict, P, ud->d_hyp_hdr, ud->d_hyp_words,
                           ud->d_hyp_hdr + (size_t)n_utt * UH_N, (const int32_t *)NULL, (const int32_t *)NULL);
        if (hipGetLastError() != hipSuccess) { s3a_set_error("s3a_uttdec_decode: ku_hyp launch failed"); rc = S3A_EHIP; }
    }
    if (rc == S3A_OK && ud->dag) rc = s3a_dagpass_enqueue(ud->dag, n_utt, ud->stream, 1);
    const size_t first_words = min((size_t)n_utt * UH_FIRST, (size_t)ud->n_lanes * ud->hyp_wcap);
    if (rc == S3A_OK && (hipMemcpyAsync(ud->h_ctx_dn, ud->S.ctx_all, sizeof(UCtx) * n_utt, hipMemcpyDeviceToHost, ud->stream) != hipSuccess
                         || hipMemcpyAsync(ud->h_hyp_hdr, ud->d_hyp_hdr, ((size_t)n_utt * UH_N + 1) * 4, hipMemcpyDeviceToHost, ud->stream) != hipSuccess
                         || hipMemcpyAsync(ud->h_hyp_words, ud->d_hyp_words, first_words * 24, hipMemcpyDeviceToHost, ud->stream) != hipSuccess)) rc = S3A_EHIP;
    if ((rc = call_close(ud, "s3a_uttdec_decode", rc, n_utt)) != S3A_OK) return rc;
    tm[3] = now();
    ud->tables_fetched = 0; ud->fstat_fetched = 0;
    for (int32_t z = 0; z < n_utt; z++) {
        const int32_t *h = ud->h_hyp_hdr + (size_t)z * UH_N;
        ud->lane[z].h_st[0] = h[UH_NENTRY]; ud->lane[z].h_st[1] = h[UH_NFRM];
    }
    {
        const size_t total_words = (size_t)ud->h_hyp_hdr[(size_t)n_utt * UH_N];
        if (total_words > first_words)
            HIPCHK(hipMemcpyAsync(ud->h_hyp_words + first_words * 6, ud->d_hyp_words + first_words * 6, (total_words - first_words) * 24,
                                  hipMemcpyDeviceToHost, ud->stream));
    }
    if (ud->dag && (rc = s3a_dagpass_finish(ud->dag, n_utt, ud->stream)) != S3A_OK) return rc;
    tm[4] = now();
    HIPCHK(hipStreamSynchronize(ud->stream));
// ... 102 lines not shown
s3a_uttdec_geometry(const s3a_uttdec_t *ud, int32_t n, int32_t *shape, int32_t *call, int32_t *engine, int32_t *frame, int32_t *window, int32_t *kf)
{
    if (!ud || n <= 0 || n > ud->n_lanes || !shape || !call || !engine || !frame || !window || !kf) return S3A_EINVAL;
    s3a_uttdec_s::FrameGeom g;
    g.fr = ug_frame(ud->shape, ud->geom, n, ud->call.hist_sort_launch);
    g.win = ug_score(ud->shape, ug_window_slots(ud->geom, n));
    const UgKf k = ug_kf(ud->shape, ud->geom, ud->call, n, ud->kf_overlapped);
    memcpy(shape, &ud->shape, sizeof ud->shape); memcpy(call, &ud->call, sizeof ud->call); memcpy(engine, &ud->geom, sizeof ud->geom);
    memcpy(frame, &g.fr, sizeof g.fr); memcpy(window, &g.win, sizeof g.win); memcpy(kf, &k, sizeof k);
    return S3A_OK;
}

static int32_t
q_keep_lattices(s3a_uttdec_t *ud, const int32_t *lanes, const int32_t *utts, int32_t n)
{
    HIPCHK(hipStreamSynchronize(ud->stream));
    for (int32_t i = 0; i < n; i++) {
        s3a_uttdec_s::QLat &q = ud->q_lat[(size_t)utts[i]];
        q.have = 0;
        if (s3a_dagpass_lattice_lane(ud->dag, lanes[i], &q.info, NULL, 0, NULL, 0) != S3A_OK) continue;
        q.nodes.resize((size_t)q.info.n_nodes + 1); q.links.resize((size_t)q.info.n_links + 1);
        if (s3a_dagpass_lattice_lane(ud->dag, lanes[i], &q.info, q.nodes.data(), q.info.n_nodes, q.links.data(), q.info.n_links) == S3A_OK) q.have = 1;
    }
    return S3A_OK;
}

static int32_t
enqueue_utts_end(s3a_uttdec_t *ud, int32_t n, const int32_t *lanes_d, const int32_t *utts_d, const int32_t *lanes_h, const int32_t *utts_h,
                 const UHypPar &P, int32_t n_utt, int32_t *wcount)
{
    int32_t rc;
    hipLaunchKernelGGL(ku_hyp, dim3(n), dim3(UH_T), 0, ud->stream, ud->d_lanes, ud->lm->d, ud->dict, P, ud->q_hdr.d, ud->q_words.d, wcount, lanes_d, utts_d);
    if (ud->dag) {
        if ((rc = s3a_dagpass_enqueue_lanes(ud->dag, lanes_d, n, ud->stream)) != S3A_OK) return rc;
        hipLaunchKernelGGL(ku_dag_store, dim3(n), dim3(UH_T), 0, ud->stream, ud->d_lanes, s3a_dagpass_dev_lanes(ud->dag), s3a_dagpass_hyp_cap(ud->dag),
                           ud->q_dio.d, ud->q_dw.d, ud->q_dio.d + (size_t)n_utt * DG_IO_N, P.wtotal, lanes_d, utts_d);
        if (ud->q_keep_lat && (rc = q_keep_lattices(ud, lanes_h, utts_h, n)) != S3A_OK) return rc;
    }
    hipLaunchKernelGGL(ku_lanes_end, dim3(8, 2 * ud->S.T, n), dim3(256), 0, ud->stream, ud->d_lanes, ud->S, lanes_d, ud->cfg.n_word);
    HIPCHK(hipGetLastError());
    return S3A_OK;
}

static int32_t
uttdec_decode_queue(s3a_uttdec_t *ud, int32_t n_utt, const float *const *feat, const int32_t *n_frames, int32_t feat_stride,
                    bool feat_on_device)
{
    if (!ud || n_utt <= 0 || !feat || !n_frames || feat_stride < ud->veclen) {
        s3a_set_error("s3a_uttdec_decode_queue: bad arguments (%d utterances)", n_utt);
        return S3A_EINVAL;
    }
    HIPCHK(hipSetDevice(ud->device));
    ud->kf_n_score = ud->kf_n_frames = ud->kf_last_c = ud->kf_n_relay = ud->kf_overlapped = 0;
    const UShared &S = ud->S;
    call_facts(ud, true, n_utt);
    int32_t route = ug_route(ud->shape, ud->geom, ud->call, 0, 0);
    const bool graph_mode = route == UG_ROUTE_GRAPH;
    const int32_t n = min(ud->n_lanes, n_utt), E = graph_mode ? graph_block_frames(ud) : (S.win_K > 0 ? S.win_K : 1), D4x4 = S.D4 * 4, T = S.T;
    int32_t rc;
    ud->n_utt = 0; ud->q_n = 0;
    ud->q_lat.clear();
    if (ud->q_keep_lat && ud->dag) { ud->q_lat.resize((size_t)n_utt); for (auto &q : ud->q_lat) q.have = 0; }
    std::vector<size_t> row0((size_t)n_utt + 1, 0);
    for (int32_t u = 0; u < n_utt; u++) {
        if (n_frames[u] <= 0 || n_frames[u] > ud->max_frames) { s3a_set_error("s3a_uttdec_decode_queue: utterance %d has %d frames (1..%d)", u, n_frames[u], ud->max_frames); return S3A_EINVAL; }
        if (!feat[u]) { s3a_set_error("s3a_uttdec_decode_queue: utterance %d has no features", u); return S3A_EINVAL; }
        row0[u + 1] = row0[u] + (size_t)n_frames[u];
    }
    KfPlan K;
    if (route == UG_ROUTE_KF_GROUPS) {
        K = kf_plan(n_utt, n_frames, KFP_LANES, (size_t)ud->n_lanes, false, 0, 0, 0, false);
        route = ug_route(ud->shape, ud->geom, ud->call, (int64_t)K.max_rows, (int64_t)sb_budget_rows(ud));
    }
    const bool kfq = route == UG_ROUTE_KF_QUEUE, kfd = route == UG_ROUTE_KF_GROUPS;
    std::vector<const float *> fd((size_t)n_utt);
    if (!feat_on_device) {
        if ((rc = q_reserve(ud, ud->q_feat, S3A_GROW_DEV | S3A_GROW_PIN, row0[n_utt] * D4x4, "features")) != S3A_OK) return rc;
        for (int32_t u = 0; u < n_utt; u++) {
            stage_features(ud, ud->q_feat.h + row0[u] * D4x4, feat[u], n_frames[u], feat_stride);
            fd[u] = ud->q_feat.d + row0[u] * D4x4;
        }
        HIPCHK(hipMemcpyAsync(ud->q_feat.d, ud->q_feat.h, row0[n_utt] * D4x4 * 4, hipMemcpyHostToDevice, ud->stream));
    }
    else {
        if (feat_stride != D4x4) { s3a_set_error("s3a_uttdec_decode_queue_dev: device features must have rows of %d floats (zero padded)", D4x4); return S3A_EINVAL; }
        for (int32_t u = 0; u < n_utt; u++) fd[u] = feat[u];
    }
    std::vector<int32_t> epoch0((size_t)n);
    for (int32_t z = 0; z < n; z++) {
        if ((rc = lane_scrub(ud, z)) != S3A_OK) return rc;
        lane_host_reset(ud->lane[z]);
        epoch0[z] = ud->lane[z].epoch;
    }
    const QSched Q = kfq ? QSched(n_utt, n) : kfd ? q_sched_groups(K, n_frames, n) : q_sched_refill(n, E, n_utt, n_frames, epoch0.data());
    if (Q.f_end < 0) return S3A_EINVAL;
    for (int32_t z = 0; z < n; z++) {
        HostLane &hl = ud->lane[z];
        hl.epoch = max(hl.epoch, Q.epoch_after[z]);
        hl.nfr = Q.nfr_after[z];
    }
    if ((rc = q_reserve(ud, ud->q_ctx, S3A_GROW_DEV | S3A_GROW_PIN, (size_t)n_utt, "contexts")) != S3A_OK) return rc;
    for (int32_t u = 0; u < n_utt; u++)
        if ((rc = utt_context(ud, ud->q_ctx.h[u], fd[u], n_frames[u], Q.epoch[u], Q.f0[u], u)) != S3A_OK) return rc;
    if ((rc = q_reserve(ud, ud->q_sched, S3A_GROW_DEV | S3A_GROW_PIN, Q.lists.size(), "schedule")) != S3A_OK) return rc;
    if (!Q.lists.empty()) {
        memcpy(ud->q_sched.h, Q.lists.data(), Q.lists.size() * 4);
// ... 149 lines not shown
    if (cluster) *cluster = ud->kf_last_c;
    return S3A_OK;
}

extern "C" int32_t
s3a_uttdec_last_relay(const s3a_uttdec_t *ud)
{
    return ud ? ud->kf_n_relay : 0;
}

extern "C" int32_t
s3a_uttdec_last_overlap(s3a_uttdec_t *ud, int32_t *overlapped, int32_t *resumed)
{
    if (!ud) return S3A_EINVAL;
    if (overlapped) *overlapped = ud->kf_overlapped;
    if (resumed) {
        *resumed = 0;
        if (ud->kf_overlapped) {
            HIPCHK(hipSetDevice(ud->device));
            HIPCHK(hipMemcpy(resumed, ud->d_kfnext + KFN_RESUMED, 4, hipMemcpyDeviceToHost));
        }
    }
    return S3A_OK;
}

extern "C" int32_t
s3a_uttdec_last_overlap2(s3a_uttdec_t *ud, int32_t *left_inside, int32_t *lead)
{
    if (!ud) return S3A_EINVAL;
    if (lead) *lead = ud->kf_overlapped ? ud->kf_lead : 0;
    if (left_inside) {
        *left_inside = 0;
        if (ud->kf_overlapped) {
            HIPCHK(hipSetDevice(ud->device));
            HIPCHK(hipMemcpy(left_inside, ud->d_kfnext + KFN_INSIDE, 4, hipMemcpyDeviceToHost));
        }
    }
    return S3A_OK;
}

extern "C" int32_t
s3a_uttdec_last_parts(s3a_uttdec_t *ud, double *score_ms, int32_t *n_score, double *frames_ms, int32_t *n_frames, int32_t *cluster)
{
    if (!ud) return S3A_EINVAL;
    if (score_ms) *score_ms = ud->kf_score_ms;
    if (frames_ms) *frames_ms = ud->kf_frames_ms;
    if (n_score) *n_score = ud->kf_n_score;
    if (n_frames) *n_frames = ud->kf_n_frames;
    if (cluster) *cluster = ud->kf_last_c;
    return S3A_OK;
}

extern "C" int32_t
s3a_uttdec_frame_dbg(s3a_uttdec_t *ud, int32_t lane, long long *out4)
{
    if (!ud || !out4 || lane < 0 || lane >= ud->n_lanes) return S3A_EINVAL;
    HIPCHK(hipSetDevice(ud->device));
    UCtx x;
    HIPCHK(hipMemcpy(&x, ud->S.ctx_all + lane, sizeof x, hipMemcpyDeviceToHost));
    for (int i = 0; i < 4; i++) out4[i] = x.kdbg[i];
    return S3A_OK;
}

extern "C" int32_t
s3a_uttdec_enable_pheur(s3a_uttdec_t *ud, int32_t pheurtype, int32_t pl_beam, int32_t pl_window, const uint8_t *const *node_ci,
                        const int16_t *sen2cimap, int32_t n_ci)
{
    if (!ud || pheurtype < 0 || pheurtype > 3) return S3A_EINVAL;
    HIPCHK(hipSetDevice(ud->device));
    if (pheurtype == 0) { ud->S.pheurtype = 0; return S3A_OK; }
    if (!node_ci || !sen2cimap || n_ci <= 0 || n_ci > PH_MAXCI || pl_window < 1) {
        s3a_set_error("s3a_uttdec_enable_pheur: bad arguments (%d CI phones, 1..%d; -pl_window %d >= 1)", n_ci, PH_MAXCI, pl_window);
        return S3A_EINVAL;
    }
    if (ud->S.n_sen <= ud->S.n_ci_sen) { s3a_set_error("s3a_uttdec_enable_pheur: the model has no CD senones"); return S3A_EUNSUP; }
    UShared &S = ud->S;
    if (!S.node_ci) {
        std::vector<uint8_t> h((size_t)S.N);
        for (int32_t t = 0; t < S.T; t++) {
            const int32_t b = ud->lane[0].ls->node_base[t], n = ud->lane[0].ls->node_base[t + 1] - b;
            if (!node_ci[t]) { s3a_set_error("s3a_uttdec_enable_pheur: no CI phones for tree %d", t); return S3A_EINVAL; }
            for (int32_t i = 0; i < n; i++) {
                if (node_ci[t][i] >= n_ci) { s3a_set_error("s3a_uttdec_enable_pheur: tree %d node %d: CI phone %d of %d", t, i, node_ci[t][i], n_ci); return S3A_EINVAL; }
                h[(size_t)b + i] = node_ci[t][i];
            }
        }
        for (int32_t j = 0; j < S.n_ci_sen; j++)
            if (sen2cimap[j] < 0 || sen2cimap[j] >= n_ci) { s3a_set_error("s3a_uttdec_enable_pheur: sen2cimap[%d] = %d", j, sen2cimap[j]); return S3A_EINVAL; }
        uint8_t *d_ci = NULL; int16_t *d_s2c = NULL;
        if (!ud->mem.dev(d_ci, (size_t)S.N) || !ud->mem.dev(d_s2c, (size_t)(S.n_ci_sen + 1) * 2)
            || hipMemcpy(d_ci, h.data(), (size_t)S.N, hipMemcpyHostToDevice) != hipSuccess
            || hipMemcpy(d_s2c, sen2cimap, (size_t)(S.n_ci_sen + 1) * 2, hipMemcpyHostToDevice) != hipSuccess) {
            ud->mem.release(d_ci); ud->mem.release(d_s2c);
            s3a_set_error("s3a_uttdec_enable_pheur: device allocation failed");
            return S3A_ENOMEM;
        }
        S.node_ci = d_ci; S.sen2cimap = d_s2c;
        std::vector<ULane> tmp((size_t)ud->n_lanes);
        for (int32_t z = 0; z < ud->n_lanes; z++) {
            ULane &u = ud->lane[z].d;
            if (!ud->mem.dev(u.ci_all, (size_t)ud->max_frames * S.n_ci_sen * 4) || !ud->mem.dev(u.heur_all, (size_t)ud->max_frames * n_ci * 4)
                || !ud->mem.dev(u.hth_pos, (size_t)3 * S.N * 4)
                || !ud->mem.dev(u.ph_scratch, ((size_t)3 * S.n_ci_sen + 8) * 4)) {
                s3a_set_error("s3a_uttdec_enable_pheur: device allocation failed");
                return S3A_ENOMEM;
            }
// ... 464 lines not shown
```

### cmusphinx_amd/lib.py

```python
from __future__ import annotations

import ctypes as C
import os

import numpy as np

HERE = os.path.dirname(os.path.abspath(__file__))
LIB_PATH = os.path.join(HERE, "libcmusphinx_amd.so")

S3A_OK = 0
LOGPROB_ZERO = -939524096
GMM_EXACT, GMM_FAST = 0, 1
MIX_INT_FLOAT_COMP = 2
MS_RAW = 1

_SIGS = {
    "s3a_last_error": (C.c_char_p, []),
    "s3a_version": (C.c_char_p, []),
    "s3a_device_count": (C.c_int32, []),
    "s3a_set_device": (C.c_int32, [C.c_int32]),
    "s3a_logmath_init": (C.c_void_p, [C.c_double, C.c_int32, C.c_int32]),
    "s3a_logs3_init": (C.c_void_p, [C.c_double, C.c_int32, C.c_int32]),
    "s3a_logmath_free": (None, [C.c_void_p]),
    "s3a_logmath_add": (C.c_int32, [C.c_void_p, C.c_int32, C.c_int32]),
# ... 139 lines not shown
    "s3a_lexsearch_hmm_histbin": (C.c_int32, [C.c_void_p, C.c_int32, C.c_int32, C.c_void_p, C.c_int32, C.c_int32]),
    "s3a_decoder_score": (C.c_int32, [C.c_void_p, C.c_void_p, C.c_int32]),
    "s3a_decoder_search": (C.c_int32, [C.c_void_p] * 3 + [C.c_int32] * 6 + [C.c_void_p] * 5 + [C.c_int32]),
    "s3a_decoder_transition": (C.c_int32, [C.c_void_p] * 3 + [C.c_int32] * 4 + [C.c_void_p] * 3 +
                               [C.c_int32, C.c_int32] + [C.c_void_p] * 3),
    "s3a_lexsearch_sen_active": (C.c_int32, [C.c_void_p, C.c_void_p, C.c_int32]),
    "s3a_lexsearch_utt_end": (C.c_int32, [C.c_void_p]),
    "s3a_lexsearch_get_active": (C.c_int32, [C.c_void_p, C.c_int32, C.c_int32, C.POINTER(C.c_int32),
                                             C.c_void_p, C.c_int32]),
    "s3a_lexsearch_get_hmm": (C.c_int32, [C.c_void_p, C.c_int32] + [C.c_void_p] * 6),
    "s3a_mgau_stream": (C.c_void_p, [C.c_void_p]),
    "s3a_scorer_sen_active_dev": (C.c_void_p, [C.c_void_p]),
    "s3a_scorer_senscr_dev": (C.c_void_p, [C.c_void_p]),
    "s3a_comsen_dev": (C.c_void_p, [C.c_void_p]),
    "s3a_approx_cont_mgau_frame_eval_dev": (C.c_int32, [C.c_void_p, C.c_void_p, C.c_void_p, C.c_int32, C.c_void_p,
                                                        C.POINTER(C.c_int32), C.POINTER(C.c_int32),
                                                        C.POINTER(C.c_int32)]),
    "s3a_lm3g_init": (C.c_void_p, [C.c_int32, C.c_void_p, C.c_void_p, C.c_void_p, C.c_int32, C.c_void_p, C.c_void_p,
                                   C.c_void_p, C.c_void_p, C.c_int32, C.c_void_p, C.c_void_p, C.c_void_p, C.c_int32]),
    "s3a_lm3g_init_host": (C.c_void_p, [C.c_int32, C.c_void_p, C.c_void_p, C.c_void_p, C.c_int32, C.c_void_p, C.c_void_p,
                                        C.c_void_p, C.c_void_p, C.c_int32, C.c_void_p, C.c_void_p, C.c_void_p, C.c_int32]),
    "s3a_lattice_nbest": (C.c_void_p, [C.c_void_p] * 7),
    "s3a_nbest_result": (C.c_int32, [C.c_void_p] * 5),
    "s3a_nbest_free": (None, [C.c_void_p]),
    "s3a_lm3g_free": (None, [C.c_void_p]),
    "s3a_lm3g_tg_score": (C.c_int32, [C.c_void_p] + [C.c_int32] * 4),
    "s3a_uttdec_init": (C.c_void_p, [C.c_void_p, C.c_void_p, C.c_void_p, C.c_int32, C.c_int32, C.c_int32, C.c_int32,
                                     C.c_double, C.c_float, C.c_int32, C.c_void_p, C.c_void_p, C.c_void_p, C.c_int32,
                                     C.c_int32, C.c_int32, C.c_int32]),
    "s3a_uttdec_init_opts": (C.c_void_p, [C.c_void_p, C.c_void_p, C.c_void_p, C.c_int32, C.c_int32, C.c_int32, C.c_int32,
                                          C.c_double, C.c_float, C.c_int32, C.c_void_p, C.c_void_p, C.c_void_p, C.c_int32,
                                          C.c_int32, C.c_int32, C.c_int32, C.c_void_p]),
    "s3a_uttdec_opts_default": (None, [C.c_void_p]),
    "s3a_uttdec_opts_from_env": (None, [C.c_void_p]),
    "s3a_uttdec_free": (None, [C.c_void_p]),
    "s3a_uttdec_decode": (C.c_int32, [C.c_void_p, C.c_int32, C.c_void_p, C.c_void_p, C.c_int32]),
    "s3a_uttdec_decode_dev": (C.c_int32, [C.c_void_p, C.c_int32, C.c_void_p, C.c_void_p, C.c_int32]),
    "s3a_uttdec_decode_queue": (C.c_int32, [C.c_void_p, C.c_int32, C.c_void_p, C.c_void_p, C.c_int32]),
    "s3a_uttdec_decode_queue_dev": (C.c_int32, [C.c_void_p, C.c_int32, C.c_void_p, C.c_void_p, C.c_int32]),
    "s3a_queue_schedule": (C.c_int32, [C.c_int32, C.c_int32, C.c_int32, C.c_void_p, C.c_void_p, C.c_void_p]),
    "s3a_queue_events": (C.c_int32, [C.c_int32] * 4 + [C.c_void_p] * 11),
    "s3a_kf_queue_plan": (C.c_int32, [C.c_int32, C.c_void_p, C.c_int32, C.c_int64] + [C.c_int32] * 5 + [C.c_void_p] * 7),
    "s3a_utt_geometry_fields": (C.c_char_p, [C.c_int32]),
    "s3a_utt_geometry": (C.c_int32, [C.c_void_p] * 2 + [C.c_int32] * 3 + [C.c_int64] * 2 + [C.c_void_p] * 7),
    "s3a_uttdec_geometry": (C.c_int32, [C.c_void_p, C.c_int32] + [C.c_void_p] * 6),
    "s3a_uttdec_queue_status": (C.c_int32, [C.c_void_p, C.c_int32, C.c_void_p, C.c_void_p, C.c_void_p, C.c_void_p]),
    "s3a_uttdec_queue_hyp": (C.c_int32, [C.c_void_p, C.c_int32, C.c_char_p, C.c_int32, C.c_void_p, C.c_void_p, C.c_int32]),
    "s3a_uttdec_result": (C.c_int32, [C.c_void_p, C.c_int32, C.c_void_p]),
    "s3a_uttdec_wl_ticks": (C.c_int32, [C.c_void_p, C.c_int32, C.c_void_p]),
    "s3a_uttdec_frame_ticks": (C.c_int32, [C.c_void_p, C.c_int32, C.c_void_p, C.c_void_p]),
    "s3a_uttdec_frame_dbg": (C.c_int32, [C.c_void_p, C.c_int32, C.c_void_p]),
    "s3a_uttdec_last_parts": (C.c_int32, [C.c_void_p] + [C.c_void_p] * 5),
    "s3a_uttdec_last_relay": (C.c_int32, [C.c_void_p]),
    "s3a_uttdec_last_overlap": (C.c_int32, [C.c_void_p, C.c_void_p, C.c_void_p]),
    "s3a_uttdec_last_overlap2": (C.c_int32, [C.c_void_p, C.c_void_p, C.c_void_p]),
    "s3a_uttdec_queue_keep_lattices": (C.c_int32, [C.c_void_p, C.c_int32]),
    "s3a_uttdec_queue_lattice": (C.c_int32, [C.c_void_p, C.c_int32, C.c_void_p, C.c_void_p, C.c_int32, C.c_void_p, C.c_int32]),
    "s3a_uttdec_n_lanes": (C.c_int32, [C.c_void_p]),
    "s3a_uttdec_window": (C.c_int32, [C.c_void_p]),
    "s3a_uttdec_enable_pheur": (C.c_int32, [C.c_void_p, C.c_int32, C.c_int32, C.c_int32, C.c_void_p, C.c_void_p, C.c_int32]),
    "s3a_uttdec_selfcheck": (C.c_int32, [C.c_void_p, C.c_int32, C.c_void_p]),
    "s3a_gather_init": (C.c_void_p, [C.c_int32, C.c_int32, C.c_char_p]),
    "s3a_get_variants": (None, [C.c_void_p]),
    "s3a_gather_init_run": (C.c_void_p, [C.c_int32, C.c_int32, C.c_char_p, C.c_uint64]),
    "s3a_gather_free": (None, [C.c_void_p]),
    "s3a_gather_hyps": (C.c_int32, [C.c_void_p, C.c_int32, C.c_void_p, C.c_void_p, C.c_int32]),
    "s3a_gather_result": (C.c_int32, [C.c_void_p, C.c_int32, C.c_void_p, C.c_void_p]),
    "s3a_dagpass_init": (C.c_void_p, [C.c_void_p, C.c_void_p, C.c_int32, C.c_int32, C.c_int32, C.c_int32, C.c_int32]),
    "s3a_dagpass_free": (None, [C.c_void_p]),
    "s3a_dagpass_run_tables": (C.c_int32, [C.c_void_p, C.c_int32, C.c_void_p]),
    "s3a_dagpass_result": (C.c_int32, [C.c_void_p, C.c_int32, C.c_void_p]),
    "s3a_dagpass_lattice": (C.c_int32, [C.c_void_p, C.c_int32, C.c_void_p, C.c_void_p, C.c_int32, C.c_void_p, C.c_int32]),
    "s3a_uttdec_lattice": (C.c_int32, [C.c_void_p, C.c_int32, C.c_void_p, C.c_void_p, C.c_int32, C.c_void_p, C.c_int32]),
    "s3a_lattice_format_s3": (C.c_int64, [C.c_char_p, C.c_void_p, C.c_void_p, C.c_void_p, C.c_void_p, C.c_void_p, C.c_int64]),
    "s3a_lattice_format_htk": (C.c_int64, [C.c_char_p, C.c_void_p, C.c_void_p, C.c_void_p, C.c_void_p, C.c_void_p, C.c_void_p, C.c_int64]),
    "s3a_uttdec_enable_bestpath": (C.c_int32, [C.c_void_p, C.c_void_p, C.c_int32, C.c_int32, C.c_int32]),
    "s3a_uttdec_bestpath_hyp": (C.c_int32, [C.c_void_p, C.c_int32, C.c_char_p, C.c_int32, C.c_void_p, C.c_void_p, C.c_int32]),
    "s3a_uttdec_bestpath_result": (C.c_int32, [C.c_void_p, C.c_int32, C.c_void_p]),
    "s3a_uttdec_queue_bestpath_hyp": (C.c_int32, [C.c_void_p, C.c_int32, C.c_char_p, C.c_int32, C.c_void_p, C.c_void_p, C.c_int32]),
    "s3a_uttdec_set_profile": (C.c_int32, [C.c_void_p, C.c_int32]),
    "s3a_uttdec_profile": (C.c_int32, [C.c_void_p, C.c_void_p, C.c_void_p, C.c_void_p, C.c_int32]),
    "s3a_variants_default": (None, [C.c_void_p]),
    "s3a_set_variants": (C.c_int32, [C.c_void_p]),
    "s3a_psfwd_init": (C.c_void_p, [C.c_void_p, C.c_int32, C.c_int32, C.c_int32, C.c_int32]),
    "s3a_psfwd_free": (None, [C.c_void_p]),
    "s3a_psfwd_n_lanes": (C.c_int32, [C.c_void_p]),
    "s3a_psfwd_start": (C.c_int32, [C.c_void_p, C.c_int32]),
    "s3a_psfwd_reset": (C.c_int32, [C.c_void_p, C.c_int32]),
    "s3a_psfwd_sen_active": (C.c_int32, [C.c_void_p, C.c_int32, C.c_int32, C.c_void_p]),
    "s3a_psfwd_step": (C.c_int32, [C.c_void_p, C.c_int32, C.c_void_p, C.c_int32, C.c_int32]),
    "s3a_psfwd_finish": (C.c_int32, [C.c_void_p, C.c_int32, C.c_int32]),
    "s3a_psfwd_set_lookahead": (C.c_int32, [C.c_void_p, C.c_int32, C.c_void_p]),
    "s3a_psfwd_decode": (C.c_int32, [C.c_void_p, C.c_void_p, C.c_int32, C.c_void_p, C.c_void_p, C.c_int32, C.c_int32]),
    "s3a_psfwd_decode_queue": (C.c_int32, [C.c_void_p, C.c_void_p, C.c_int32, C.c_void_p, C.c_void_p, C.c_int32]),
    "s3a_psfwd_queue_hyp": (C.c_int32, [C.c_void_p, C.c_int32, C.POINTER(C.c_int32), C.c_void_p, C.c_int32]),
    "s3a_psfwd_table": (C.c_int32, [C.c_void_p, C.c_int32, C.c_void_p]),
    "s3a_psfwd_hyp": (C.c_int32, [C.c_void_p, C.c_int32, C.POINTER(C.c_int32), C.c_void_p, C.c_int32]),
    "s3a_psfwd_get_sp_ssid": (C.c_int32, [C.c_void_p, C.c_int32, C.c_void_p]),
    "s3a_psfwd_set_sp_ssid": (C.c_int32, [C.c_void_p, C.c_int32, C.c_void_p]),
    "s3a_psfwd_last_decode_ms": (C.c_double, [C.c_void_p]),
    "s3a_psfwd_last_score_ms": (C.c_double, [C.c_void_p]),
    "s3a_uttdec_shape": (C.c_int32, [C.c_void_p] + [C.POINTER(C.c_int32)] * 6),
    "s3a_uttdec_hyp": (C.c_int32, [C.c_void_p, C.c_int32, C.c_char_p, C.c_int32, C.c_void_p]),
    "s3a_uttdec_hyp_var": (C.c_int32, [C.c_void_p, C.c_int32, C.c_char_p, C.c_int32, C.c_void_p, C.c_void_p, C.c_int32]),
    "s3a_hyp_format_var": (C.c_int32, [C.c_void_p, C.c_void_p, C.c_void_p, C.c_void_p, C.c_void_p, C.c_int32, C.c_int32, C.c_float,
                                       C.c_int32, C.c_int32, C.c_char_p, C.c_size_t, C.c_char_p, C.c_size_t]),
# ... 1330 lines not shown
        for k in ("frame_start", "bestscore", "bestvh"):
            out[k] = np.ctypeslib.as_array(getattr(r, k), (nf + 1,)).copy()
        out["frame_stat"] = np.ctypeslib.as_array(r.frame_stat, (r.n_frames * 8,)).reshape(-1, 8).copy()
        out.update(err=r.err, n_frm=nf, max_cand=r.max_cand, max_new=r.max_new, n_tie_frames=r.n_tie_frames)
        return out

    def set_profile(self, every):
        check(self.L.s3a_uttdec_set_profile(self.h, int(every)), self.L)

    def profile(self):
        us = (C.c_double * 24)(); n = (C.c_int64 * 24)(); names = (C.c_char_p * 24)()
        k = self.L.s3a_uttdec_profile(self.h, us, n, names, 24)
        return {names[i].decode(): (us[i], n[i]) for i in range(k) if n[i]}

    def wl_ticks(self, lane=0):
        t = (C.c_longlong * 16)()
        check(self.L.s3a_uttdec_wl_ticks(self.h, int(lane), t), self.L)
        return [0.01 * t[i] for i in range(9)]

    def frame_ticks(self, lane=0):
        t = (C.c_longlong * 16)(); c = C.c_int32()
        check(self.L.s3a_uttdec_frame_ticks(self.h, int(lane), t, C.byref(c)), self.L)
        names = ("enter_test", "enter_rank", "enter_apply_mark", "comsen_mark", "select", "comsen_max", "hmm_eval", "stamp_hist", "weak",
                 "resolve", "scan", "emit_word")
        d = {names[i]: 0.01 * t[i] for i in range(12)}
        d["emit_only"] = 0.01 * t[15]; d["in_launch"] = 0.01 * t[12]
        return d, int(t[13]), int(t[14]), int(c.value)

    def last_parts(self):
        sm, fm = C.c_double(), C.c_double()
        ns, nf, c = C.c_int32(), C.c_int32(), C.c_int32()
        check(self.L.s3a_uttdec_last_parts(self.h, C.byref(sm), C.byref(ns), C.byref(fm), C.byref(nf), C.byref(c)), self.L)
        return dict(score_ms=sm.value, n_score=ns.value, frames_ms=fm.value, n_frames=nf.value, cluster=c.value)

    def geometry(self, n):
        out = {k: _geom_out(r) for k, r in (("shape", "shape"), ("call", "call"), ("engine", "engine"), ("frame", "frame"),
                                            ("window", "score"), ("kf", "kf"))}
        check(self.L.s3a_uttdec_geometry(self.h, int(n), *[_p(a) for a in out.values()]), self.L)
        return {k: _geom_dict("score" if k == "window" else k, a) for k, a in out.items()}

    def last_overlap(self):
        o, r = C.c_int32(), C.c_int32()
        check(self.L.s3a_uttdec_last_overlap(self.h, C.byref(o), C.byref(r)), self.L)
        return dict(overlapped=o.value, resumed=r.value)

    def last_overlap2(self):
        n, l = C.c_int32(), C.c_int32()
        check(self.L.s3a_uttdec_last_overlap2(self.h, C.byref(n), C.byref(l)), self.L)
        return dict(left_inside=n.value, lead=l.value)

    def last_relay(self):
        return int(self.L.s3a_uttdec_last_relay(self.h))

    def frame_dbg(self, lane=0):
        t = (C.c_longlong * 4)()
        check(self.L.s3a_uttdec_frame_dbg(self.h, int(lane), t), self.L)
        return [int(x) for x in t]

    def hyp(self, lane, uttid="", utt_index=0):
        rec = HypRecord()
        check(self.L.s3a_uttdec_hyp(self.h, lane, uttid.encode(), int(utt_index), C.byref(rec)), self.L)
        return rec

    def window(self):
        return int(self.L.s3a_uttdec_window(self.h))

    def enable_pheur(self, pheurtype, pl_beam, pl_window, node_ci, sen2cimap, n_ci):
        arrs = [np.ascontiguousarray(a, np.uint8) for a in node_ci]
        ptrs = (C.c_void_p * len(arrs))(*[a.ctypes.data for a in arrs])
        s2c = np.ascontiguousarray(sen2cimap, np.int16)
        check(self.L.s3a_uttdec_enable_pheur(self.h, int(pheurtype), int(pl_beam), int(pl_window), ptrs, _p(s2c), int(n_ci)), self.L)

    def selfcheck(self, lane):
        out = np.zeros(8, np.int32)
        check(self.L.s3a_uttdec_selfcheck(self.h, int(lane), _p(out)), self.L)
        return out

    def enable_bestpath(self, cfg, link_cap=0, pair_cap=0, keep_tables=True):
        self._dag_cfg = cfg
        check(self.L.s3a_uttdec_enable_bestpath(self.h, C.byref(cfg), int(link_cap), int(pair_cap), 1 if keep_tables else 0), self.L)

    def bestpath_result(self, lane):
        r = DagResult()
        check(self.L.s3a_uttdec_bestpath_result(self.h, int(lane), C.byref(r)), self.L)
        return r

    def bestpath_hyp(self, lane, uttid="", utt_index=0):
        hdr = HypHeader()
        words = np.zeros((HYP_MAXW, 6), np.int32)
        check(self.L.s3a_uttdec_bestpath_hyp(self.h, lane, uttid.encode(), int(utt_index), C.byref(hdr), _p(words), len(words)), self.L)
        if hdr.status == -3:
            words = np.zeros((hdr.n_words, 6), np.int32)
            check(self.L.s3a_uttdec_bestpath_hyp(self.h, lane, uttid.encode(), int(utt_index), C.byref(hdr), _p(words), len(words)), self.L)
        return hdr, words[:hdr.n_words if hdr.status == 0 else 0].copy()

    def _lattice(self, fn, k):
        info = LatInfo()
        check(fn(self.h, int(k), C.byref(info), None, 0, None, 0), self.L)
        nodes, links = np.zeros((info.n_nodes, 6), np.int32), np.zeros((max(info.n_links, 1), 5), np.int32)
        check(fn(self.h, int(k), C.byref(info), _p(nodes), info.n_nodes, _p(links), info.n_links), self.L)
        return info, nodes, links[:info.n_links]

    def lattice(self, lane):
        return self._lattice(self.L.s3a_uttdec_lattice, lane)

    def queue_keep_lattices(self, on=True):
# ... 28 lines not shown
```

### include/cmusphinx_amd.h

```cpp
#ifndef CMUSPHINX_AMD_H
#define CMUSPHINX_AMD_H

#include <stdint.h>
#include <stddef.h>

#ifdef __cplusplus
extern "C" {
#endif

#define S3A_OK        0
#define S3A_EINVAL   (-1)
#define S3A_EIO      (-2)
#define S3A_ENOMEM   (-3)
#define S3A_ENODEV   (-4)
#define S3A_EHIP     (-5)
#define S3A_EUNSUP   (-6)

#define S3A_LOGPROB_ZERO  ((int32_t)0xc8000000)
#define S3A_MAX_NEG_INT32 ((int32_t)0x80000000)
#define S3A_NO_BSTIDX   (-1)
#define S3A_NOT_UPDATED (-100)
#define S3A_FULL_INT_COMP      0
#define S3A_FULL_FLOAT_COMP    1
#define S3A_MIX_INT_FLOAT_COMP 2
// ... 343 lines not shown
s3a_uttdec_t *s3a_uttdec_init(const s3a_lexsearch_t *proto, s3a_mgau_model_t *g, const int16_t *cd2cisen,
                              int32_t n_sen, int32_t n_ci_sen, int32_t ds_ratio, int32_t cond_ds,
                              double ci_pbeam, float tighten_factor, int32_t max_cd, s3a_comsen_t *cs,
                              s3a_lm3g_t *lm, const s3a_wordlevel_cfg_t *cfg, int32_t n_lanes,
                              int32_t max_frames, int32_t vh_cap, int32_t cand_cap);
typedef struct {
    int32_t many, big_wl, window, framecheck, times;
    int32_t graph;
    int32_t scan_small_from;
    int32_t persist;
    int32_t cluster;
    int32_t score_rows_max;
    int32_t reserved[1];
} s3a_uttdec_opts_t;
void s3a_uttdec_opts_default(s3a_uttdec_opts_t *o);
void s3a_uttdec_opts_from_env(s3a_uttdec_opts_t *o);
s3a_uttdec_t *s3a_uttdec_init_opts(const s3a_lexsearch_t *proto, s3a_mgau_model_t *g, const int16_t *cd2cisen,
                                   int32_t n_sen, int32_t n_ci_sen, int32_t ds_ratio, int32_t cond_ds, double ci_pbeam,
                                   float tighten_factor, int32_t max_cd, s3a_comsen_t *cs, s3a_lm3g_t *lm,
                                   const s3a_wordlevel_cfg_t *cfg, int32_t n_lanes, int32_t max_frames, int32_t vh_cap,
                                   int32_t cand_cap, const s3a_uttdec_opts_t *opts);
void s3a_uttdec_free(s3a_uttdec_t *ud);
int32_t s3a_uttdec_decode(s3a_uttdec_t *ud, int32_t n_utt, const float *const *feat,
                          const int32_t *n_frames, int32_t feat_stride);
int32_t s3a_uttdec_decode_dev(s3a_uttdec_t *ud, int32_t n_utt, const float *const *feat_dev,
                              const int32_t *n_frames, int32_t feat_stride);
int32_t s3a_uttdec_result(s3a_uttdec_t *ud, int32_t lane, s3a_utt_result_t *out);
int32_t s3a_uttdec_decode_queue(s3a_uttdec_t *ud, int32_t n_utt, const float *const *feat,
                                const int32_t *n_frames, int32_t feat_stride);
int32_t s3a_uttdec_decode_queue_dev(s3a_uttdec_t *ud, int32_t n_utt, const float *const *feat_dev,
                                    const int32_t *n_frames, int32_t feat_stride);
int32_t s3a_uttdec_queue_status(s3a_uttdec_t *ud, int32_t utt, int32_t *err, int32_t *stopped_at,
                                int32_t *max_cand, int32_t *max_new);
int32_t s3a_queue_schedule(int32_t n_lanes, int32_t boundary, int32_t n_utt, const int32_t *n_frames,
                           int32_t *lane, int32_t *f0);
int32_t s3a_queue_events(int32_t groups, int32_t n_lanes, int32_t boundary, int32_t n_utt, const int32_t *n_frames, const int32_t *epoch0,
                         int32_t *sizes, int32_t *lane, int32_t *f0, int32_t *epoch, int32_t *last_utt, int32_t *epoch_after,
                         int32_t *nfr_after, int32_t *events, int32_t *lists);
int32_t s3a_kf_queue_plan(int32_t n_utt, const int32_t *n_frames, int32_t rule, int64_t budget, int32_t in_order, int32_t n1,
                          int32_t lead_groups, int32_t round_groups, int32_t whole, int64_t *sizes, int32_t *order, int32_t *cut,
                          int64_t *row0, int64_t *g_at, int64_t *groups, int64_t *steps);
const char *s3a_utt_geometry_fields(int32_t record);
int32_t s3a_utt_geometry(const int32_t *shape, const int32_t *call, int32_t n, int32_t ov, int32_t score_slots, int64_t max_rows,
                         int64_t budget, int32_t *engine, int32_t *frame, int32_t *window, int32_t *score, int32_t *companion,
                         int32_t *kf, int32_t *route);
int32_t s3a_uttdec_geometry(const s3a_uttdec_t *ud, int32_t n, int32_t *shape, int32_t *call, int32_t *engine, int32_t *frame, int32_t *window,
                            int32_t *kf);
int32_t s3a_uttdec_wl_ticks(s3a_uttdec_t *ud, int32_t lane, long long *out16);
int32_t s3a_uttdec_last_parts(s3a_uttdec_t *ud, double *score_ms, int32_t *n_score, double *frames_ms, int32_t *n_frames, int32_t *cluster);
int32_t s3a_uttdec_last_overlap(s3a_uttdec_t *ud, int32_t *overlapped, int32_t *resumed);
int32_t s3a_uttdec_last_overlap2(s3a_uttdec_t *ud, int32_t *left_inside, int32_t *lead);
int32_t s3a_uttdec_frame_ticks(s3a_uttdec_t *ud, int32_t lane, long long *out16, int32_t *cluster);
int32_t s3a_uttdec_last_relay(const s3a_uttdec_t *ud);
int32_t s3a_uttdec_frame_dbg(s3a_uttdec_t *ud, int32_t lane, long long *out4);
int32_t s3a_uttdec_n_lanes(const s3a_uttdec_t *ud);
int32_t s3a_uttdec_selfcheck(s3a_uttdec_t *ud, int32_t lane, int32_t *out8);
int32_t s3a_uttdec_window(const s3a_uttdec_t *ud);
int32_t s3a_uttdec_enable_pheur(s3a_uttdec_t *ud, int32_t pheurtype, int32_t pl_beam, int32_t pl_window,
                                const uint8_t *const *node_ci, const int16_t *sen2cimap, int32_t n_ci);
#define S3A_HYP_MAXW 250
typedef struct { int32_t wid, sf, ef, ascr, lscr, scale; } s3a_hyp_word_t;
typedef struct {
    char uttid[96];
    int32_t utt_index, n_words, n_frames, score, total_scale, n_entry, status, exit_id;
    s3a_hyp_word_t word[S3A_HYP_MAXW];
} s3a_hyp_record_t;
int32_t s3a_uttdec_hyp(s3a_uttdec_t *ud, int32_t lane, const char *uttid, int32_t utt_index,
                       s3a_hyp_record_t *rec);
int32_t s3a_hyp_format(const s3a_hyp_record_t *rec, const char *const *wordstr, const int32_t *basewid,
                       const uint8_t *is_filler, int32_t startwid, int32_t finishwid, float lw, int32_t wip,
                       int32_t unscale, char *match_line, size_t match_cap, char *seg_line, size_t seg_cap);
typedef struct {
    char uttid[96];
    int32_t utt_index, n_words, n_frames, score, total_scale, n_entry, status, exit_id;
} s3a_hyp_header_t;
int32_t s3a_uttdec_hyp_var(s3a_uttdec_t *ud, int32_t lane, const char *uttid, int32_t utt_index,
                           s3a_hyp_header_t *hdr, s3a_hyp_word_t *words, int32_t max_words);
int32_t s3a_uttdec_queue_hyp(s3a_uttdec_t *ud, int32_t utt, const char *uttid, int32_t utt_index,
                             s3a_hyp_header_t *hdr, s3a_hyp_word_t *words, int32_t max_words);
int32_t s3a_hyp_format_var(const s3a_hyp_header_t *hdr, const s3a_hyp_word_t *words, const char *const *wordstr,
                           const int32_t *basewid, const uint8_t *is_filler, int32_t startwid, int32_t finishwid,
                           float lw, int32_t wip, int32_t unscale, char *match_line, size_t match_cap,
                           char *seg_line, size_t seg_cap);

typedef struct s3a_wltest_s s3a_wltest_t;
s3a_wltest_t *s3a_wltest_init(s3a_lm3g_t *lm, const s3a_wordlevel_cfg_t *cfg, const int32_t *lcmap_len,
                              int32_t vh_cap, int32_t cand_cap, int32_t max_exits, int32_t max_frames);
void s3a_wltest_free(s3a_wltest_t *wt);
int32_t s3a_wltest_begin(s3a_wltest_t *wt, int32_t startwid, int32_t n_frames);
int32_t s3a_wltest_frame(s3a_wltest_t *wt, const int32_t *n_exit, const int32_t *exits, int32_t best_hmm,
                         int32_t best_word, int32_t word_thres, int32_t *n_calls, int32_t *calls,
                         int32_t *thresh, int32_t *n_ent);
int32_t s3a_wltest_fetch(s3a_wltest_t *wt, int32_t *n_entry, int32_t *n_frm, int32_t *out,
                         int32_t max_entries, int32_t *frames, int32_t max_out_frames,
                         int32_t *n_tie_frames);

typedef struct s3a_gather_s s3a_gather_t;
s3a_gather_t *s3a_gather_init(int32_t rank, int32_t world, const char *rendezvous);
s3a_gather_t *s3a_gather_init_run(int32_t rank, int32_t world, const char *rendezvous, unsigned long long run_id);
void s3a_gather_free(s3a_gather_t *g);
int32_t s3a_gather_hyps(s3a_gather_t *g, int32_t n_local, const s3a_hyp_header_t *hdr, const s3a_hyp_word_t *words,
                        int32_t n_total);
int32_t s3a_gather_result(const s3a_gather_t *g, int32_t utt_index, const s3a_hyp_header_t **hdr,
                          const s3a_hyp_word_t **words);

typedef struct s3a_dagpass_s s3a_dagpass_t;
// ... 188 lines not shown
```

Baseline: 803,000 frames/s.

## Stage senone score row in LDS early for select and comsen max

When the senone row fits in LDS and dynamic CI beam is off, the row is prefetched with vector loads into registers before the entry-reset loop, written to LDS, and then used by a new LDS-based select pass and by the comsen max reduction, which reads LDS instead of global memory. Select metadata (cd2cisen, best index, ncomp) is packed and prefetched one iteration ahead. Backed-off senones rewritten during select are counted across workgroups, and when any occurred in a multi-workgroup lane the row is reloaded from global. This removes repeated global reads of the score row at the cost of extra registers, another cross-workgroup counter, and some gate statistics plumbing exposed to the host.

```diff
diff --git a/cmusphinx_amd/csrc/s3a_decoder_kernels.h b/cmusphinx_amd/csrc/s3a_decoder_kernels.h
--- a/cmusphinx_amd/csrc/s3a_decoder_kernels.h
+++ b/cmusphinx_amd/csrc/s3a_decoder_kernels.h
@@ -1298,7 +1298,7 @@
     }
 }
 
-template <bool MAXOP, int U = 4>
+template <bool MAXOP, int U = 4, bool LDSRAW = false>
 __device__ __forceinline__ void
 d_comsen_list(const int32_t *__restrict__ wl, int32_t n_w, const int32_t *__restrict__ cs_off, const int16_t *__restrict__ cs_list,
               uint8_t *sen_active, const int32_t *__restrict__ raw, int32_t *cs_val, int32_t grp, int32_t n_grp,
@@ -1327,7 +1327,11 @@
 #pragma unroll
                 for (int h = 0; h < 2; h++)
                 {
-                    if (MAXOP) { const int32_t x = ((const __attribute__((address_space(1))) int32_t *)raw)[max(id[u][h], 0)]; if (id[u][h] >= 0) mx[u] = max(mx[u], x); }
+                    if (MAXOP) {
+                        const int32_t x = LDSRAW ? ((const __attribute__((address_space(3))) int32_t *)raw)[max(id[u][h], 0)]
+                                                 : ((const __attribute__((address_space(1))) int32_t *)raw)[max(id[u][h], 0)];
+                        if (id[u][h] >= 0) mx[u] = max(mx[u], x);
+                    }
                     else if (id[u][h] >= 0) { if (actbits) (void)__hip_atomic_fetch_or((__attribute__((address_space(3))) uint32_t *)&actbits[id[u][h] >> 5], 1u << (id[u][h] & 31), __ATOMIC_RELAXED, __HIP_MEMORY_SCOPE_WORKGROUP); else sen_active[id[u][h]] = 1; }
                 }
         }
diff --git a/cmusphinx_amd/csrc/s3a_utt.hip b/cmusphinx_amd/csrc/s3a_utt.hip
--- a/cmusphinx_amd/csrc/s3a_utt.hip
+++ b/cmusphinx_amd/csrc/s3a_utt.hip
@@ -60,6 +60,7 @@
     UCtx *ctx;
     int32_t *pack;
     WLane w;
+    int32_t *gate_bo;
 };
 
 struct UShared {
@@ -730,6 +731,103 @@
     }
 }
 
+__device__ __forceinline__ int32_t
+d_select_fetch(const UShared &S, const uint8_t *brow, int32_t sen)
+{
+    const int32_t sq = sen < S.n_sen ? sen : S.n_ci_sen;
+    return ((int32_t)GMC(S.cd2cisen)[sq] & 0xffff) | ((int32_t)GMC(brow)[sq] << 16) | ((int32_t)GMC(S.ncomp)[sq] << 24);
+}
+
+template <bool EXACT, int NT>
+__device__ __forceinline__ void
+d_select_lds(const ULane &L, const UShared &S, const UCtx *ctx, int32_t f, int32_t *row, int32_t *rowl, const uint8_t *brow, int32_t bx, int32_t G,
+             const uint32_t *actbits, int32_t cig_part, int32_t (&pk)[4], int32_t *n_bo)
+{
+    __shared__ int32_t red[4][NT / 64];
+    const int32_t tid = threadIdx.x, ln = tid & 63;
+    int32_t pb = INT_MIN;
+    for (int32_t ci = ln; ci < S.n_ci_sen; ci += 64) pb = max(pb, LM(rowl)[ci]);
+#pragma unroll
+    for (int o = 32; o > 0; o >>= 1) pb = max(pb, __shfl_xor(pb, o, 64));
+    if (tid < 64 && bx == 0) {
+        int32_t cig = cig_part;
+#pragma unroll
+        for (int o = 32; o > 0; o >>= 1) cig += __shfl_xor(cig, o, 64);
+        if (tid == 0) { L.misc[5] = pb; L.misc[3] = S.n_ci_sen; L.misc[4] = cig; }
+    }
+    const int32_t is_skip = (f % S.ds_ratio == 0) ? 0 : 1;
+    const int32_t thresh = add32(pb, is_skip ? S.ci_pbeam_tight : S.ci_pbeam);
+    LogAdd la;
+    la.tab = S.tab16; la.size = S.tab_size; la.zero = S.lm_zero;
+    int32_t rbest = INT_MIN, rns = 0, rng = 0, rbo = 0;
+    const int32_t step = 4 * G * NT;
+    for (int32_t s0 = S.n_ci_sen + bx * NT; s0 < S.n_sen; s0 += step) {
+        int32_t pkn[4];
+#pragma unroll
+        for (int u = 0; u < 4; u++) pkn[u] = d_select_fetch(S, brow, s0 + step + u * G * NT + tid);
+        int32_t senq[4], cisq[4], rowq[4], obq[4], utq[4];
+        bool actq[4];
+        bool out = false;
+#pragma unroll
+        for (int u = 0; u < 4; u++) {
+            const int32_t sen = s0 + u * G * NT + tid;
+            const bool in = sen < S.n_sen;
+            senq[u] = in ? sen : S.n_ci_sen;
+            actq[u] = in && ((LM(actbits)[senq[u] >> 5] >> (senq[u] & 31)) & 1u) != 0;
+            cisq[u] = LM(rowl)[pk[u] & 0xffff]; rowq[u] = LM(rowl)[senq[u]];
+            obq[u] = S3A_NO_BSTIDX; utq[u] = 0;
+            out = out || (actq[u] && cisq[u] < thresh);
+        }
+        if (__ballot(out)) {
+#pragma unroll
+            for (int u = 0; u < 4; u++) { obq[u] = GMC(L.bstidx)[senq[u]]; utq[u] = GMC(L.updatetime)[senq[u]]; }
+        }
+#pragma unroll
+        for (int u = 0; u < 4; u++) {
+            if (!actq[u]) continue;
+            const int32_t sen = senq[u];
+            const int32_t ci_scr = cisq[u];
+            if (ci_scr >= thresh) {
+                const int32_t bi = (pk[u] >> 16) & 0xff;
+                GM(L.bstidx)[sen] = bi == 255 ? S3A_NO_BSTIDX : bi;
+                GM(L.updatetime)[sen] = f;
+                rbest = max(rbest, rowq[u]); rns++; rng += (int32_t)((uint32_t)pk[u] >> 24);
+                continue;
+            }
+            rbo++;
+            const int32_t bi = obq[u], ut = utq[u];
+            if (bi == S3A_NO_BSTIDX || ut != f - 1) {
+                GM(row)[sen] = ci_scr; ((S3A_AS3 int32_t *)rowl)[sen] = ci_scr;
+                rbest = max(rbest, ci_scr);
+                continue;
+            }
+            const int32_t v = uw_one_gaussian<EXACT>(S, sen * S.CP + bi, ctx->feat + (size_t)f * S.D4 * 4);
+            int32_t score = la(S3A_LOGPROB_ZERO, v);
+            if (score <= S3A_LOGPROB_ZERO) score = S3A_LOGPROB_ZERO;
+            GM(row)[sen] = score; ((S3A_AS3 int32_t *)rowl)[sen] = score;
+            rbest = max(rbest, score); rng++;
+            if (is_skip) { L.bstidx[sen] = v > S3A_LOGPROB_ZERO ? bi : S3A_NO_BSTIDX; L.updatetime[sen] = f; }
+        }
+#pragma unroll
+        for (int u = 0; u < 4; u++) pk[u] = pkn[u];
+    }
+#pragma unroll
+    for (int o = 32; o > 0; o >>= 1) {
+        rbest = max(rbest, __shfl_xor(rbest, o, 64)); rns += __shfl_xor(rns, o, 64); rng += __shfl_xor(rng, o, 64); rbo += __shfl_xor(rbo, o, 64);
+    }
+    if (ln == 0) { red[0][tid >> 6] = rbest; red[1][tid >> 6] = rns; red[2][tid >> 6] = rng; red[3][tid >> 6] = rbo; }
+    __syncthreads();
+    if (tid == 0) {
+        for (int w = 1; w < NT / 64; w++) { rbest = max(rbest, red[0][w]); rns += red[1][w]; rng += red[2][w]; rbo += red[3][w]; }
+        if (bx < S.gp_n) {
+            L.gpart[bx] = rbest;
+            L.gpart[S.gp_n + bx] = rns;
+            L.gpart[2 * S.gp_n + bx] = rng;
+        }
+        *n_bo = rbo;
+    }
+}
+
 template <bool EXACT>
 __global__ void __launch_bounds__(256)
 ku_select(const ULane *__restrict__ lanes, UShared S, int32_t fg, int32_t K)
@@ -1404,6 +1502,8 @@
     int32_t ps_exact;
     uint32_t psbits[KF_PSBITS / 32];
     long long kacc[16];
+    int32_t gacc[4];
+    int32_t gate_bo;
     int32_t thr[4];
     int32_t tp[KF_TP_LDS];
     struct { const void *A; UCtx *ctx; int32_t *row; const uint8_t *brow; int32_t *bar_cnt; int32_t z, r, C, f, weak, bar_target, bar_local; } fa;
@@ -1437,6 +1537,7 @@
     int32_t *n_resumed;
     const int32_t *f_ready;
     int32_t *n_inside;
+    unsigned long long *gate;
 };
 
 __device__ __forceinline__ void
@@ -1676,6 +1777,7 @@
     if (f == 0) {
         for (int32_t i = tid; i < KF_SENBITS / 32; i += KF_NT) sh.senbits[i] = 0u;
         if (C > 1 && r == 0) for (int32_t i = tid; i < KF_SENBITS / 32; i += KF_NT) L.senbits[i] = 0u;
+        if (C > 1 && r == 0 && tid == 0) L.gate_bo[0] = 0;
         kf_barrier(B);
     }
 
@@ -1878,6 +1980,18 @@
         for (int32_t t = 0; t < T; t++) { sh.pre[t] = a; a += nact_cur[t]; }
         sh.pre[T] = a;
     }
+    constexpr int KF_ROWQ = (int)((sizeof(KfPool) / 16 + KF_NT - 1) / KF_NT);
+    const int32_t gsel_all = max(1, min(USEL_G, min(S.gp_n, (S.n_sen - S.n_ci_sen + 255) / 256))), gsel = min(C, gsel_all);
+    const bool dyn = S.max_cd < S.n_sen - S.n_ci_sen;
+    const bool row_fits = (size_t)S.n_sen * 4 <= sizeof(KfPool), row_early = row_fits && !dyn;
+    const bool row_v4 = row_early && ((unsigned long long)row & 15ull) == 0 && S.n_sen >= 4;
+    int32_t *const row_lds = (int32_t *)&sh.pool;
+    s3a_v4i rq[KF_ROWQ];
+    if (row_v4) {
+        const int32_t n4 = S.n_sen >> 2;
+#pragma unroll
+        for (int q = 0; q < KF_ROWQ; q++) { const int32_t i = q * KF_NT + tid; rq[q] = ((const S3A_AS1 s3a_v4i *)row)[i < n4 ? i : 0]; }
+    }
     if (n_ent > 0) {
         const int32_t R = (((n_ent + gwaves - 1) / gwaves) + 63) & ~63, P = sh.seg[gwaves];
         for (int32_t i = gtid; i < P; i += gstride) {
@@ -1887,12 +2001,27 @@
             L.key[v] = 0ull; L.first[v] = INT_MAX;
         }
     }
+    if (row_early) {
+        const int32_t n4 = row_v4 ? S.n_sen >> 2 : 0;
+        if (row_v4) {
+#pragma unroll
+            for (int q = 0; q < KF_ROWQ; q++) { const int32_t i = q * KF_NT + tid; if (i < n4) ((S3A_AS3 s3a_v4i *)row_lds)[i] = rq[q]; }
+        }
+        for (int32_t i = 4 * n4 + tid; i < S.n_sen; i += KF_NT) row_lds[i] = row[i];
+    }
     const int32_t n_csw = S3A_ALD(&L.cs_wn[0]);
 #ifndef KF_CSU
 #define KF_CSU 4
 #endif
     d_comsen_list<false, KF_CSU>(L.cs_wl, n_csw, S.cs_off, S.cs_list, (uint8_t *)NULL, (const int32_t *)NULL, (int32_t *)NULL, gtid >> 4, gstride >> 4,
                          (const int32_t *)NULL, sh.senbits);
+    int32_t g_pk[4], g_cig = 0;
+    if (row_early && r < gsel) {
+#pragma unroll
+        for (int u = 0; u < 4; u++) g_pk[u] = d_select_fetch(S, brow, S.n_ci_sen + r * KF_NT + u * gsel * KF_NT + tid);
+        if (r == 0 && tid < 64) for (int32_t ci = tid; ci < S.n_ci_sen; ci += 64) g_cig += (int32_t)GMC(S.ncomp)[ci];
+        if (tid == 0) sh.gate_bo = 0;
+    }
     if (C > 1) {
         __syncthreads();
         for (int32_t i = tid; i < KF_SENBITS / 32; i += KF_NT) if (sh.senbits[i]) atomicOr(&L.senbits[i], sh.senbits[i]);
@@ -1906,18 +2035,30 @@
     const int32_t n_tot = sh.pre[T];
     const bool hist_frame = n_tot > bm.maxhmmpf + (bm.maxhmmpf >> 1);
     {
-        const int32_t g_all = max(1, min(USEL_G, min(S.gp_n, (S.n_sen - S.n_ci_sen + 255) / 256))), G = min(C, g_all);
-        const bool dyn = S.max_cd < S.n_sen - S.n_ci_sen;
+        const int32_t g_all = gsel_all, G = gsel;
         if (dyn && r < G) kf_dyn_ci_beam<KF_NT>(S, f, row, sh.senbits, (int32_t *)&sh.pool, &sh.dynbeam);
         if (dyn && r == 0 && tid == 0) L.dynbeam[0] = sh.dynbeam;
-        if (r < G) d_select<EXACT, KF_NT>(L, S, ctx, f, row, brow, r, G, sh.senbits, dyn ? &sh.dynbeam : (const int32_t *)NULL);
+        if (row_early) {
+            if (r < G) {
+                d_select_lds<EXACT, KF_NT>(L, S, ctx, f, row, row_lds, brow, r, G, sh.senbits, g_cig, g_pk, &sh.gate_bo);
+                if (C > 1 && tid == 0 && sh.gate_bo > 0) atomicAdd(L.gate_bo, sh.gate_bo);
+            }
+        }
+        else if (r < G) d_select<EXACT, KF_NT>(L, S, ctx, f, row, brow, r, G, sh.senbits, dyn ? &sh.dynbeam : (const int32_t *)NULL);
         if (r == 0 && tid >= G && tid < g_all) { L.gpart[tid] = INT_MIN; L.gpart[S.gp_n + tid] = 0; L.gpart[2 * S.gp_n + tid] = 0; }
     }
     kf_barrier(B);
+    const int32_t n_bo = !row_early ? 0 : C > 1 ? S3A_ALD(L.gate_bo) : sh.gate_bo;
+    if (C > 1 && n_bo > 0) {
+        for (int32_t i = tid; i < S.n_sen; i += KF_NT) row_lds[i] = GMC(row)[i];
+        __syncthreads();
+    }
+    if (r == 0 && tid == 0) { sh.gacc[0]++; if (n_bo > 0) { sh.gacc[1]++; sh.gacc[2] += n_bo; } }
     for (int32_t i = tid; i < KF_SENBITS / 32; i += KF_NT) sh.senbits[i] = 0u;
     if (C > 1 && r == 0) for (int32_t i = tid; i < KF_SENBITS / 32; i += KF_NT) L.senbits[i] = 0u;
     KF_STAMP(4);
-    d_comsen_list<true, KF_CSU>(L.cs_wl, n_csw, S.cs_off, S.cs_list, (uint8_t *)NULL, row, L.cs_val, gtid >> 4, gstride >> 4, S.cs_wt);
+    if (row_early) d_comsen_list<true, KF_CSU, true>(L.cs_wl, n_csw, S.cs_off, S.cs_list, (uint8_t *)NULL, row_lds, L.cs_val, gtid >> 4, gstride >> 4, S.cs_wt);
+    else d_comsen_list<true, KF_CSU>(L.cs_wl, n_csw, S.cs_off, S.cs_list, (uint8_t *)NULL, row, L.cs_val, gtid >> 4, gstride >> 4, S.cs_wt);
     kf_barrier(B);
     KF_STAMP(5);
     {
@@ -1928,9 +2069,9 @@
         if (lane == 0) sh.red[wave] = gb;
         if (tid < 2 * T) sh.acc[tid] = INT_MIN;
         if (r == 0 && tid == 0) L.cs_wn[0] = 0;
-        const bool row_in_lds = (size_t)S.n_sen * 4 <= sizeof(KfPool);
-        int32_t *row_lds = (int32_t *)&sh.pool;
-        if (row_in_lds)
+        if (C > 1 && r == 0 && tid == 0) L.gate_bo[0] = 0;
+        const bool row_in_lds = row_fits;
+        if (row_fits && !row_early)
             for (int32_t i = tid; i < S.n_sen; i += KF_NT) row_lds[i] = row[i];
         __syncthreads();
         int32_t norm = max(L.misc[0], L.misc[5]);
@@ -2539,6 +2680,8 @@
     UCtx *ctx = S.ctx_all + z;
     if (tid == 0) { sh.dead = 0; sh.fk = J.f_ready ? 0 : INT32_MAX; }
     if (tid < 16) sh.kacc[tid] = 0;
+    if (tid < 4) sh.gacc[tid] = 0;
+#define KF_GATE_FLUSH() do { if (r == 0 && tid < 4 && J.gate && sh.gacc[tid]) { atomicAdd(&J.gate[tid], (unsigned long long)sh.gacc[tid]); sh.gacc[tid] = 0; } } while (0)
     for (int32_t i = tid; i < KF_SENBITS / 32; i += KF_NT) sh.senbits[i] = 0u;
     if (tid <= S.T) sh.nb[tid] = S.node_base[tid];
     if (S.n_tmat * NS_TPW(NE) <= KF_TP_LDS)
@@ -2593,7 +2736,7 @@
             if (u < 0) {
                 if (tid == 0) { sh.kacc[12] += (long long)wall_clock64() - t_launch; sh.kacc[14]++; }
                 __syncthreads();
-                if (tid < 16) { ctx->kacc[tid] += sh.kacc[tid]; sh.kacc[tid] = 0; }
+                if (tid < 16) { ctx->kacc[tid] += sh.kacc[tid]; sh.kacc[tid] = 0; } KF_GATE_FLUSH();
                 if (tid == 0 && J.ov == 1) {
                     ctx->kdbg[0] = t_launch; ctx->kdbg[1] = (long long)wall_clock64();
                     ctx->kdbg[2] = (long long)__builtin_amdgcn_s_getreg((31 << 11) | 4); ctx->kdbg[3] = (long long)__builtin_amdgcn_s_getreg((31 << 11) | 20);
@@ -2642,7 +2785,7 @@
                     if (f >= F) {
                         if (tid == 0) { sh.kacc[12] += (long long)wall_clock64() - t_launch; sh.kacc[14]++; J.lane_f[z] = f; }
                         __syncthreads();
-                        if (tid < 16) { ctx->kacc[tid] += sh.kacc[tid]; sh.kacc[tid] = 0; }
+                        if (tid < 16) { ctx->kacc[tid] += sh.kacc[tid]; sh.kacc[tid] = 0; } KF_GATE_FLUSH();
                         if (tid == 0 && J.ov == 1) {
                             ctx->kdbg[0] = t_launch; ctx->kdbg[1] = (long long)wall_clock64();
                             ctx->kdbg[2] = (long long)__builtin_amdgcn_s_getreg((31 << 11) | 4); ctx->kdbg[3] = (long long)__builtin_amdgcn_s_getreg((31 << 11) | 20);
@@ -2688,6 +2831,7 @@
         if (handed) break;
         if (mode != KF_QUEUE) break;
         if (r == 0 && tid < 16 && tid != 12 && tid != 14) { ctx->kacc[tid] += sh.kacc[tid]; sh.kacc[tid] = 0; }
+        KF_GATE_FLUSH();
         static_assert(3 * WL_LDS_EX >= UH_IDS, "d_hyp's backtrace ids borrow the word level's exit area");
         if (r == 0) d_hyp<KF_NT>(L, ctx, lm, dict, J.P, J.hdr + (size_t)u * UH_N, J.words, J.wcount, sh.pool.wl.ex);
         kf_barrier(B);
@@ -2700,6 +2844,8 @@
     }
     if (r == 0 && tid == 0) { sh.kacc[12] += (long long)wall_clock64() - t_launch; sh.kacc[14]++; }
     if (r == 0 && tid < 16) ctx->kacc[tid] += sh.kacc[tid];
+    KF_GATE_FLUSH();
+#undef KF_GATE_FLUSH
     if (r == 0 && tid == 0 && ((J.mode == KF_WINDOW && J.fg0 == 512) || J.ov == 1 || (J.ov == 2 && z >= J.n1))) {
         ctx->kdbg[0] = t_launch; ctx->kdbg[1] = (long long)wall_clock64();
         ctx->kdbg[2] = (long long)__builtin_amdgcn_s_getreg((31 << 11) | 4); ctx->kdbg[3] = (long long)__builtin_amdgcn_s_getreg((31 << 11) | 20);
@@ -3047,6 +3193,7 @@
     int32_t kf_last_c;
     int32_t kf_counted;
     int32_t *d_kfnext;
+    unsigned long long *d_kfgate;
     void *d_kfargs, *h_kfargs;
     int32_t kf_arg_at;
     s3a_grow<int32_t> sb_scores; s3a_grow<uint8_t> sb_bests;
@@ -3378,6 +3525,8 @@
         DM(ud->mem, ud->d_kfnext, (size_t)(KFN_LANE + n_lanes) * 4);
         DM(ud->mem, ud->d_kfargs, sizeof(KfArgs) * KF_ARG_SLOTS);
         if (!ud->mem.pin(ud->h_kfargs, sizeof(KfArgs) * KF_ARG_SLOTS)) { s3a_set_error("s3a_uttdec_init: pinned allocation failed"); goto fail; }
+        DM(ud->mem, ud->d_kfgate, 4 * sizeof(unsigned long long));
+        if (hipMemset(ud->d_kfgate, 0, 4 * sizeof(unsigned long long)) != hipSuccess) goto fail;
         DM(ud->mem, ud->d_kfbar, (size_t)n_lanes * 8);
         if (hipMemset(ud->d_kfbar, 0, (size_t)n_lanes * 8) != hipSuccess) goto fail;
         DM(ud->mem, ud->d_kfrelay, ((size_t)(KF_STAGES + 1) * (KF_ST_WORDS + n_lanes) + (size_t)3 * n_lanes) * 4);
@@ -3421,6 +3570,7 @@
         DM(ud->mem, u.cs_need, (size_t)(cs->n_comstate + 1) * 4); DM(ud->mem, u.cs_val, (size_t)(cs->n_comstate + 1) * 4); DM(ud->mem, u.dynbeam, 16);
         DM(ud->mem, u.cs_wl, (size_t)(cs->n_comstate + 1) * 4); DM(ud->mem, u.cs_wn, 16); u.ent = ls->d_ent; DM(ud->mem, u.posbest, (size_t)(proto->N + 64) * 4); DM(ud->mem, u.posps, (size_t)(proto->N + 64) * 4);
         DM(ud->mem, u.senbits, KF_SENBITS / 8); if (hipMemset(u.senbits, 0, KF_SENBITS / 8) != hipSuccess) goto fail;
+        DM(ud->mem, u.gate_bo, 16); if (hipMemset(u.gate_bo, 0, 16) != hipSuccess) goto fail;
         if (hipMemset(u.cs_wn, 0, 16) != hipSuccess) goto fail; DM(ud->mem, u.pstamp8, (size_t)proto->n_pset + 64); S.n_pset_bytes = proto->n_pset + 64;
         DM(ud->mem, u.plist, (size_t)(proto->N + 64) * 4); DM(ud->mem, u.pcnt, 16); DM(ud->mem, u.claim, (size_t)(proto->N + 64) * 4);
         if (hipMemset(u.pcnt, 0, 16) != hipSuccess) goto fail;
@@ -3779,7 +3929,7 @@
     if (rc != S3A_OK) return rc;
     KfJob J;
     memset(&J, 0, sizeof J);
-    J.mode = KF_WINDOW; J.fg0 = fg0; J.n_fr = nf;
+    J.mode = KF_WINDOW; J.fg0 = fg0; J.n_fr = nf; J.gate = ud->d_kfgate;
     ud->kf_n_score++; ud->kf_n_frames++;
     return kf_launch_c(ud, n, J, ug_kf_choose_c(ud->shape, ud->geom, kf_alone(ud), n));
 }
@@ -3884,7 +4034,7 @@
     kf_mark(ud);
     KfJob J;
     memset(&J, 0, sizeof J);
-    J.mode = KF_STATIC; J.row0 = row0; J.scores = ud->sb_scores.d; J.bests = ud->sb_bests.d;
+    J.mode = KF_STATIC; J.gate = ud->d_kfgate; J.row0 = row0; J.scores = ud->sb_scores.d; J.bests = ud->sb_bests.d;
     if ((rc = kf_launch_chain(ud, m, J)) != S3A_OK) return rc;
     ud->kf_n_frames++;
     kf_mark(ud);
@@ -3953,7 +4103,7 @@
         else HIPCHK(hipMemsetAsync(ud->d_kfnext + KFN_COUNTER, 0, 4, ud->stream));
         KfJob J;
         memset(&J, 0, sizeof J);
-        J.mode = KF_QUEUE; J.n_utt = nu; J.u0 = u0; J.order = ud->kf_order.d; J.next = ud->d_kfnext + KFN_COUNTER; J.lane_u = ud->d_kfnext + KFN_LANE; J.stage = ud->q_ctx.d;
+        J.mode = KF_QUEUE; J.gate = ud->d_kfgate; J.n_utt = nu; J.u0 = u0; J.order = ud->kf_order.d; J.next = ud->d_kfnext + KFN_COUNTER; J.lane_u = ud->d_kfnext + KFN_LANE; J.stage = ud->q_ctx.d;
         J.row0 = ud->sb_row0.d; J.scores = ud->sb_scores.d; J.bests = ud->sb_bests.d;
         J.hdr = ud->q_hdr.d; J.words = ud->q_words.d; J.wcount = wcount; J.P = P; J.B = B; J.n_word = ud->cfg.n_word;
         if ((rc = kf_launch_chain(ud, min(ud->n_lanes, nu), J, n1 > 0 ? &K : NULL)) != S3A_OK) return rc;
@@ -4187,6 +4337,7 @@
     int32_t rc, maxT = 0;
     ud->q_n = 0;
     ud->kf_n_score = ud->kf_n_frames = ud->kf_last_c = ud->kf_n_relay = ud->kf_overlapped = 0;
+    if (ud->d_kfgate) HIPCHK(hipMemsetAsync(ud->d_kfgate, 0, 4 * sizeof(unsigned long long), ud->stream));
     double tm[6] = { 0, 0, 0, 0, 0, 0 };
     auto now = []() { struct timespec ts; clock_gettime(CLOCK_MONOTONIC, &ts); return ts.tv_sec + 1e-9 * ts.tv_nsec; };
     tm[0] = now();
@@ -4395,6 +4546,7 @@
     }
     HIPCHK(hipSetDevice(ud->device));
     ud->kf_n_score = ud->kf_n_frames = ud->kf_last_c = ud->kf_n_relay = ud->kf_overlapped = 0;
+    if (ud->d_kfgate) HIPCHK(hipMemsetAsync(ud->d_kfgate, 0, 4 * sizeof(unsigned long long), ud->stream));
     const UShared &S = ud->S;
     call_facts(ud, true, n_utt);
     int32_t route = ug_route(ud->shape, ud->geom, ud->call, 0, 0);
@@ -4650,6 +4802,20 @@
 }
 
 extern "C" int32_t
+s3a_uttdec_last_gate(s3a_uttdec_t *ud, long long *out4)
+{
+    if (!ud || !out4) return S3A_EINVAL;
+    for (int i = 0; i < 4; i++) out4[i] = 0;
+    if (!ud->d_kfgate) return S3A_OK;
+    HIPCHK(hipSetDevice(ud->device));
+    HIPCHK(hipStreamSynchronize(ud->stream));
+    unsigned long long g[4];
+    HIPCHK(hipMemcpy(g, ud->d_kfgate, sizeof g, hipMemcpyDeviceToHost));
+    for (int i = 0; i < 4; i++) out4[i] = (long long)g[i];
+    return S3A_OK;
+}
+
+extern "C" int32_t
 s3a_uttdec_frame_dbg(s3a_uttdec_t *ud, int32_t lane, long long *out4)
 {
     if (!ud || !out4 || lane < 0 || lane >= ud->n_lanes) return S3A_EINVAL;
diff --git a/cmusphinx_amd/lib.py b/cmusphinx_amd/lib.py
--- a/cmusphinx_amd/lib.py
+++ b/cmusphinx_amd/lib.py
@@ -215,6 +215,7 @@
     "s3a_uttdec_frame_dbg": (C.c_int32, [C.c_void_p, C.c_int32, C.c_void_p]),
     "s3a_uttdec_last_parts": (C.c_int32, [C.c_void_p] + [C.c_void_p] * 5),
     "s3a_uttdec_last_relay": (C.c_int32, [C.c_void_p]),
+    "s3a_uttdec_last_gate": (C.c_int32, [C.c_void_p, C.c_void_p]),
     "s3a_uttdec_last_overlap": (C.c_int32, [C.c_void_p, C.c_void_p, C.c_void_p]),
     "s3a_uttdec_last_overlap2": (C.c_int32, [C.c_void_p, C.c_void_p, C.c_void_p]),
     "s3a_uttdec_queue_keep_lattices": (C.c_int32, [C.c_void_p, C.c_int32]),
@@ -1651,6 +1652,11 @@
     def last_relay(self):
         return int(self.L.s3a_uttdec_last_relay(self.h))
 
+    def last_gate(self):
+        t = (C.c_longlong * 4)()
+        check(self.L.s3a_uttdec_last_gate(self.h, t), self.L)
+        return dict(frames=int(t[0]), backoff_frames=int(t[1]), backoffs=int(t[2]), rewalks=int(t[3]))
+
     def frame_dbg(self, lane=0):
         t = (C.c_longlong * 4)()
         check(self.L.s3a_uttdec_frame_dbg(self.h, int(lane), t), self.L)
diff --git a/include/cmusphinx_amd.h b/include/cmusphinx_amd.h
--- a/include/cmusphinx_amd.h
+++ b/include/cmusphinx_amd.h
@@ -419,6 +419,7 @@
 int32_t s3a_uttdec_last_overlap2(s3a_uttdec_t *ud, int32_t *left_inside, int32_t *lead);
 int32_t s3a_uttdec_frame_ticks(s3a_uttdec_t *ud, int32_t lane, long long *out16, int32_t *cluster);
 int32_t s3a_uttdec_last_relay(const s3a_uttdec_t *ud);
+int32_t s3a_uttdec_last_gate(s3a_uttdec_t *ud, long long *out4);
 int32_t s3a_uttdec_frame_dbg(s3a_uttdec_t *ud, int32_t lane, long long *out4);
 int32_t s3a_uttdec_n_lanes(const s3a_uttdec_t *ud);
 int32_t s3a_uttdec_selfcheck(s3a_uttdec_t *ud, int32_t lane, int32_t *out8);
```

Measured after the change: 805,500 frames/s, median of 4. About the same (+0.3%).
